# eanswer/TactileSimulation

Hardware: AMD Instinct MI355X
Metric: env-steps/sec (fwd+bwd) TactilePush batch=4096 (higher is better)
Workload: dtype f32

## Files before the change

include/tsim.h:

```cpp
#ifndef TSIM_H
#define TSIM_H
#include <stdint.h>
#ifdef __cplusplus
extern "C" {
#endif

typedef struct tsim_batch tsim_batch;
enum { TSIM_F32 = 0, TSIM_F64 = 1 };

int tsim_batch_create(const int32_t* I, const double* F, int B, int tape_capacity, int dtype, int device,
                      tsim_batch** out);
void tsim_batch_destroy(tsim_batch* b);

int tsim_ndof_r(const tsim_batch* b);
int tsim_ndof_u(const tsim_batch* b);
int tsim_ndof_var(const tsim_batch* b);
int tsim_ndof_tactile(const tsim_batch* b);
int tsim_batch_size(const tsim_batch* b);
int tsim_dtype(const tsim_batch* b);
double tsim_timestep(const tsim_batch* b);
int tsim_tape_len(const tsim_batch* b);

int tsim_update_model(tsim_batch* b, const int32_t* I, const double* F, void* stream);

int tsim_set_env_tables(tsim_batch* b, const void* tables, void* stream);
int tsim_table_size(const tsim_batch* b);

int tsim_set_param_grad(tsim_batch* b, void* dL_dtables);

enum { TSIM_PG_CONTACT = 1, TSIM_PG_INERTIAL = 2, TSIM_PG_MOTOR = 4, TSIM_PG_LIMIT = 8 };
int tsim_set_param_grad_groups(tsim_batch* b, int mask);
int tsim_get_param_grad_groups(const tsim_batch* b);

enum { TSIM_ADJ_BACKWARD = 0, TSIM_ADJ_BACKWARD_Z = 1, TSIM_ADJ_CLOSED_BACKWARD_Z = 2 };
int tsim_last_adjoint_launch(const tsim_batch* b, int32_t* out);

int tsim_reset(tsim_batch* b, const void* q0, const void* qd0, int backward_flag, void* stream);

int tsim_reset_masked(tsim_batch* b, const void* q0, const void* qd0, const int32_t* mask, void* stream);

int tsim_step(tsim_batch* b, const void* u, int num_steps, void* q_out, void* qd_out, void* var_out,
              void* tac_out, int32_t* status, void* stream);

int tsim_get_state(tsim_batch* b, void* q_out, void* qd_out, void* stream);
int tsim_readout(tsim_batch* b, void* var_out, void* tac_out, void* stream);

int tsim_backward_steps(tsim_batch* b, int n, int seed_mode, const void* df_dq, const void* df_dvar,
                        const void* df_dtac, void* df_du, void* stream);

int tsim_rollout(tsim_batch* b, const void* u, int num_frames, int num_steps, const int32_t* tactile_slot,
                 void* q_out, void* qd_out, void* var_out, void* tac_out, int32_t* status, void* stream);

int tsim_backward_episode(tsim_batch* b, int num_frames, int num_steps, const int32_t* tactile_slot,
                          const void* df_dq, const void* df_dvar, const void* df_dtac, void* df_du, void* stream);

enum { TSIM_TANGENT_MAX_DIR = 8 };
int tsim_tangent_episode(tsim_batch* b, int num_frames, int num_steps, int ndir, const int32_t* tactile_slot,
                         const void* du, const void* dq0, const void* dqd0, const void* dtables,
                         void* dq_out, void* dqd_out, void* dvar_out, void* dtac_out, void* stream);
int tsim_tangent_launch_info(const tsim_batch* b, int ndir, int with_dtables, int32_t* out);

int tsim_frame_jacobians(tsim_batch* b, int num_frames, int num_steps, void* A_out, void* B_out, void* Jvar_out, void* stream);
int tsim_frame_jacobians_launch_info(const tsim_batch* b, int32_t* out);

int tsim_tactile_jacobians(tsim_batch* b, int num_frames, int num_steps, const int32_t* tactile_slot, void* Ct_out, void* stream);
int tsim_tactile_jacobians_launch_info(const tsim_batch* b, int32_t* out);

enum { TSIM_PARAM_JACOBIAN_MAX_COLS = 32 };
int tsim_param_jacobians(tsim_batch* b, int num_frames, int num_steps, int ncols, const int32_t* cols,
                         const int32_t* tactile_slot, void* E_out, void* Ft_out, void* stream);
int tsim_param_jacobians_launch_info(const tsim_batch* b, int32_t* out);

int tsim_get_adjoint(tsim_batch* b, void* df_dq0, void* df_dqd0, void* stream);

int tsim_cache_save(tsim_batch* b, void* stream);
int tsim_cache_pop(tsim_batch* b, void* stream);
int tsim_cache_clear(tsim_batch* b);
int tsim_cache_reserve(tsim_batch* b, int depth);
int tsim_cache_depth(const tsim_batch* b);

int tsim_debug_eval(tsim_batch* b, const void* q1, const void* q0, const void* qd0, const void* u,
                    void* g_out, void* H_out, long long* cycles, void* stream);

int tsim_debug_signature(tsim_batch* b, int t_first, int n, uint32_t* out, void* stream);

int tsim_debug_stamps(tsim_batch* b, long long* cycles);

int tsim_launch_info(const tsim_batch* b, int32_t* out);
enum { TSIM_KT_FORWARD = 0, TSIM_KT_TAXELS = 1, TSIM_KT_BACKWARD = 2, TSIM_KT_COUNT = 3 };
int tsim_kernel_timing(tsim_batch* b, int enable);
int tsim_kernel_times(tsim_batch* b, double* ms_sum, int32_t* launches);
int tsim_set_lanes_per_env(tsim_batch* b, int lanes);
int tsim_static_model(const tsim_batch* b);
int tsim_set_static(tsim_batch* b, int allow);
const char* tsim_kernel_variant(const tsim_batch* b);
enum { TSIM_OPT_PAIR_CULL = 1, TSIM_OPT_VALUE_TRIALS = 2, TSIM_OPT_TRIAL_HELPERS = 3, TSIM_OPT_VALUE_FIRST = 4, TSIM_OPT_CROSS_KINKS = 5, TSIM_OPT_EVAL_BUDGET = 6,
       TSIM_OPT_ALL_DEFAULT = 7, TSIM_OPT_FRAME_RECORDS = 8, TSIM_OPT_FORWARD_SPLIT = 9 };
int tsim_set_option(tsim_batch* b, int option, int value);
int tsim_get_option(const tsim_batch* b, int option);

int tsim_last_evals(tsim_batch* b, int32_t* host_out);
int tsim_last_helper_trials(tsim_batch* b, int32_t* host_out);

#define TSIM_KINK_FACTOR 1000.0
#define TSIM_KINK_LS 4
#define TSIM_KINK_MAX 6
int tsim_set_solver_options(tsim_batch* b, int cross_kinks, int eval_budget);
int tsim_last_gnorm(tsim_batch* b, float* host_out);

const char* tsim_last_error(void);

#ifdef __cplusplus
}
#endif
#endif
```

tactilesimulation_amd/csrc/tsim_batch.h:

```cpp
#pragma once
#include <hip/hip_runtime.h>
#include <cstdint>
#include <string>
#include <vector>
#include "../../include/tsim.h"
#include "tsim_launch.h"

static thread_local std::string g_err;
static int fail(const std::string& m) { g_err = m; return 1; }
#define HIPCHK(x) do { hipError_t e_ = (x); if (e_ != hipSuccess) return fail(std::string(#x) + ": " + hipGetErrorString(e_)); } while (0)

struct DeviceGuard {
  int prev = -1; bool ok = true;
  explicit DeviceGuard(int dev) {
    if (hipGetDevice(&prev) != hipSuccess) prev = -1;
    if (prev != dev) ok = hipSetDevice(dev) == hipSuccess; else prev = -1;
  }
  ~DeviceGuard() { if (prev >= 0) (void)hipSetDevice(prev); }
};
#define TS_DEVICE(b) DeviceGuard guard_((b)->device); if (!guard_.ok) return fail("hipSetDevice(" + std::to_string((b)->device) + ") failed")

static bool capturing(hipStream_t st) {
  hipStreamCaptureStatus cs = hipStreamCaptureStatusNone;
  return hipStreamIsCapturing(st, &cs) != hipSuccess || cs != hipStreamCaptureStatusNone;
}

template <class F> static auto by_dtype(int dtype, F&& f) { return dtype == TSIM_F32 ? f(float()) : f(double()); }

struct DevBuf {
  void* p = nullptr;
  DevBuf() = default;
  DevBuf(const DevBuf&) = delete;
  DevBuf& operator=(const DevBuf&) = delete;
  ~DevBuf() { (void)hipFree(p); }
  template <class U> operator U*() const { return static_cast<U*>(p); }
  explicit operator bool() const { return p != nullptr; }
  void** operator&() { return &p; }
  void* take() { void* q = p; p = nullptr; return q; }
  void release() { (void)hipFree(take()); }
};

struct CacheEntry { void* buf; int len; int record, tape_k_ok; };
struct KtPair { hipEvent_t a, b; int kind; };
struct tsim_batch {
  int B, dtype, device, cap;
  std::vector<int32_t> I; std::vector<double> F;
  int nl, nr, nu, nvar, ntax, rec;
  int tape_k = 0, tape_k_ok = 0;
  DevBuf dI, dF;
  DevBuf dFenv; int nfrec;
  void* tape = nullptr;
  DevBuf lamq, lamv;
  DevBuf evals;
  DevBuf helped;
  DevBuf gnorm;
  int cross_kinks = 0, eval_budget = 0;
  DevBuf order; int order_valid = 0;
  DevBuf order_ep; int order_ep_n = 0;
  DevBuf prev; int has_prev = 0;
  DevBuf poseR, poseD; int nspt;
  int has_exp;
  int t_cur, record;
  int lpe_forced;
  int nsched;
  int stage_cpt;
  int n_simd;
  int last_frame_rec = 0;
  hipStream_t split_st = nullptr;
  hipEvent_t split_fork = nullptr;
  hipEvent_t split_join = nullptr;
  int last_fwd_split = 0;
  int value_trials = 2;
  int trial_helpers = 1;
  int value_first = 1;
  bool ab_no_episode_lpt = false, ab_inkernel_readout = false, ab_no_free_run = false, ab_lockstep = false, ab_taxels_per_record = false, ab_no_envtab_cpt = false, ab_no_default_opts = false, ab_inkernel_frame_out = false; int ab_bwd_lpe = 0, ab_lpt_deal = 2;
  int pair_cull = 1;
  int static_id = 0, static_exact = 0, env_struct_ok = 0, no_static = 0;
  DevBuf dKmask, dFlag;
  DevBuf fposeR, fposeD; int fpose_frames = 0;
  int pose_valid = 0;
  int pose_off = 0;
  int tt_off = 0;
  int tax_slots = 0;
  size_t esz;
  std::vector<CacheEntry> cache;
  std::vector<void*> pool;
  std::vector<void*> retired;
  long long* bwd_stamps = nullptr;
  void* dLdp = nullptr; DevBuf zbuf, pgpart; int pg_chunks = 0;
  int pg_groups = TS_PG_CONTACT; DevBuf pgbpart;
  DevBuf tan_src; size_t tan_src_reals = 0; int tan_src_captured = 0;
  DevBuf pg_slots;
  int adj_kernel = -1, adj_passes = 0;
  int kt_on = 0;
  std::vector<KtPair> kt;
  std::vector<hipEvent_t> kt_free;
};
template <class F> static auto by_real(const tsim_batch* b, F&& f) { return by_dtype(b->dtype, f); }
static void split_release(tsim_batch* b) {
  if (b->split_st) (void)hipStreamDestroy(b->split_st);
  if (b->split_fork) (void)hipEventDestroy(b->split_fork);
  if (b->split_join) (void)hipEventDestroy(b->split_join);
  b->split_st = nullptr; b->split_fork = b->split_join = nullptr;
}

struct KtScope {
  tsim_batch* b; hipStream_t st; KtPair p; bool on = false;
  KtScope(tsim_batch* b_, int kind, hipStream_t st_) : b(b_), st(st_) {
    if (!b->kt_on || b->kt.size() >= (size_t)1 << 16) return;
    if (capturing(st)) return;
    hipEvent_t e[2];
    for (int i = 0; i < 2; ++i) {
      if (!b->kt_free.empty()) { e[i] = b->kt_free.back(); b->kt_free.pop_back(); }
      else if (hipEventCreate(&e[i]) != hipSuccess) { (void)hipGetLastError(); if (i) b->kt_free.push_back(e[0]); return; }
    }
    p.a = e[0]; p.b = e[1]; p.kind = kind;
    on = hipEventRecord(p.a, st) == hipSuccess;
    if (!on) { b->kt_free.push_back(e[0]); b->kt_free.push_back(e[1]); }
  }
  ~KtScope() { if (on) { (void)hipEventRecord(p.b, st); b->kt.push_back(p); } }
};

struct GrowWant { DevBuf& buf; size_t bytes; };
static int grow_buffers(tsim_batch* b, hipStream_t st, bool named, std::initializer_list<GrowWant> want) {
  HIPCHK(hipStreamSynchronize(st));
  for (const GrowWant& w : want) {
    if (!named) w.buf.release();
    else if (w.buf) b->retired.push_back(w.buf.take());
  }
  for (const GrowWant& w : want)
    if (hipMalloc(&w.buf, w.bytes) != hipSuccess) {
      (void)hipGetLastError();
      for (const GrowWant& v : want) v.buf.release();
      return -1;
    }
  return 0;
}

static int plan_info(const TsPlan& p, int32_t* out) {
  out[0] = (int32_t)p.lds; out[1] = TS_WAVE; out[2] = (int32_t)p.grid; out[3] = p.lpe;
  return 0;
}
```

tactilesimulation_amd/csrc/tsim_hip.hip:

```cpp
#include <hip/hip_runtime.h>
#include <cstdio>
#include <cstdlib>
#include <cstring>
#include <cmath>
#include <algorithm>
#include <string>
#include <vector>
#include "../../include/tsim.h"
#include "tsim_eval.h"
#include "tsim_policy_push.h"
#include "tsim_static_pusher.h"


#include "tsim_kernels.h"
#include "tsim_param_grad.h"
#include "tsim_launch.h"
#include "tsim_batch.h"

__global__ void __launch_bounds__(1024) k_order_by_evals(const int* evals, int* order, int B, int ns, int lo, int span, int deal) {
  __shared__ int hist[64], base[64];
  const int t = threadIdx.x;
  if (t < 64) hist[t] = 0;
  __syncthreads();
  auto bin = [lo, span](int ev) { return min(max((ev - lo) * 64 / span, 0), 63); };
// ... 20 lines not shown
  const int env = blockIdx.x, lane = threadIdx.x;
  Ctx<R> c; ctx_init(c, a.I, a.F, lds, 1, 0, lane, TS_WAVE, a.stage_cpt != 0, a.Fenv ? a.Fenv + (size_t)blockIdx.x * a.fstride : nullptr);
  const int nr = c.nr, REC = ts_rec(nr, c.nu, (int)sizeof(R), a.tk);
  init_world(c, lane, TS_WAVE);
  const R* st = a.tape + ((size_t)a.t0 * a.B + env) * REC;
  if (lane < nr) { c.qD[lane] = rec_q(st)[lane]; c.q[lane] = (R)c.qD[lane]; c.qd[lane] = st[rec_qd<R>(nr) + lane]; c.qa[lane] = R(0); }
  TS_SYNC();
  phase1<R, false, true>(c, lane, R(0), R(0), R(0));
  readout<TS_WAVE>(c, lane, env, true, false, a.var_out != nullptr, false, a.var_out, (R*)nullptr);
  if (!a.poseR) return;
  int k = 0;
  for (int s = 0; s < c.nsensor; ++s) {
    const int* si = c.I + c.off_sensor + s * TSIM_SI_SIZE;
    for (int j = 0; j < si[TSIM_SI_NSPRIM]; ++j, ++k) {
      TS_SYNC();
      pair_stage_value(c, c.I[c.off_sprim + si[TSIM_SI_SPRIM0] + j], 0, lane == 0);
      TS_SYNC();
      const size_t rec = (size_t)env * a.nspt + k;
      if (lane < TP_R_SIZE) a.poseR[rec * TP_R_SIZE + lane] = c.PP[lane];
      if (lane < TP_D_SIZE) a.poseD[rec * TP_D_SIZE + lane] = c.PPd[lane];
    }
  }
}

template <class R> struct TaxArgs { const int* I; const R* F; const R* Fenv; int fstride; const R* poseR; const double* poseD; int nspt; R* tac_out; int slice;
  int B; const int* tac_slot;
  int ntax, nsensor, foff_sensor, foff_pair, foff_taxel, tt_off; };

enum { TX_MAXS = 16, TX_MAXK = 64 };
template <class R> __device__ __forceinline__ void ts_store3(R* o, R a, R b, R c) {
  __builtin_nontemporal_store(a, o); __builtin_nontemporal_store(b, o + 1); __builtin_nontemporal_store(c, o + 2);
}
template <class R>
__device__ __forceinline__ void taxel_eval(int t, V3<R> xa, int nsensor, const int* sEnd, const int* sKb, const int* sNsp, const int* sPrim, const R* sSf,
                                           const R* sShape, const R* sP, const double* sD, const R* sC, const R* tax, int ntax, R* out) {
  int s = 0;
  while (s < nsensor - 1 && t >= sEnd[s]) ++s;
  const int kb = sKb[s], nsp = sNsp[s];
  const R* sf = sSf + s * TSIM_SF_SIZE;
  const R* tp = tax + t;
  V3<R> Fl = zero3<R>();
  for (int j = 0; j < nsp; ++j) {
    const R* Cc = sC + (kb + j) * 4;
    const V3<R> dc = xa - ldv(Cc);
    if (Cc[3] >= R(0) && dot3(dc, dc) > Cc[3]) continue;
    const int prim = sPrim[kb + j];
    const R* shape = sShape + (kb + j) * 4;
    const R* P = sP + (kb + j) * TP_R_SIZE;
    const double* D = sD + (kb + j) * TP_D_SIZE;
    const M3<R> RPA = ldm(P);
    if (sizeof(R) == 4 && !(prim_distance<R>(prim, shape, mulMv(RPA, xa) + ldv(P + 9)) < R(TS_FAR_MARGIN))) continue;
    const V3<double> xPd = mulMv(ldm(D), cvt3<double>(xa)) + ldv(D + 9);
    const V3<R> xP = cvt3<R>(xPd);
    V3<R> Fc; M3<R> Jx, Jv;
    if (contact_law<R, false>(prim, shape, sf, xP, ldv(P + 15) + cross3(ldv(P + 12), xP), Fc, Jx, Jv, xPd)) Fl = Fl + mulMtv(RPA, Fc);
  }
  R o0 = R(0), o1 = R(0), o2 = R(0);
  if (Fl.x != R(0) || Fl.y != R(0) || Fl.z != R(0)) {
    o0 = Fl.x * tp[3 * ntax] + Fl.y * tp[4 * ntax] + Fl.z * tp[5 * ntax];
    o1 = Fl.x * tp[6 * ntax] + Fl.y * tp[7 * ntax] + Fl.z * tp[8 * ntax];
    o2 = Fl.x * tp[9 * ntax] + Fl.y * tp[10 * ntax] + Fl.z * tp[11 * ntax];
  }
  ts_store3(out + 3 * t, o0, o1, o2);
}
template <class R> __device__ __forceinline__ void taxel_bound(const R* P, int prim, const R* sh, R* C) {
  const V3<R> cA = mulMtv(ldm(P), ldv(P + 9)) * R(-1);
  R rb = R(-1);
  if (prim == TSIM_P_SPHERE) rb = sh[0];
  else if (prim == TSIM_P_CUBOID) rb = t_sqrt(sh[0] * sh[0] + sh[1] * sh[1] + sh[2] * sh[2]);
  else if (prim == TSIM_P_CYLINDER) rb = t_sqrt(sh[0] * sh[0] + sh[1] * sh[1]);
  C[0] = cA.x; C[1] = cA.y; C[2] = cA.z;
  C[3] = rb < R(0) ? R(-1) : (rb + R(TS_FAR_MARGIN)) * (rb + R(TS_FAR_MARGIN));
}
enum { TS_TAX_UNROLL = 2 };
template <class R>
__global__ void __launch_bounds__(256) k_taxels(TaxArgs<R> a) {
  const int rec_env = blockIdx.x, env = rec_env % a.B, frame = rec_env / a.B;
  const int tslot = a.tac_slot ? a.tac_slot[frame] : frame;
  if (tslot < 0) return;
  const int* I = a.I;
  const R* F = a.Fenv ? a.Fenv + (size_t)env * a.fstride : a.F;
  const int ntax = a.ntax, nsensor = a.nsensor;
  __shared__ int sEnd[TX_MAXS], sKb[TX_MAXS], sNsp[TX_MAXS], sPrim[TX_MAXK];
  __shared__ R sSf[TX_MAXS * TSIM_SF_SIZE], sShape[TX_MAXK * 4], sP[TX_MAXK * TP_R_SIZE];
  __shared__ double sD[TX_MAXK * TP_D_SIZE];
  __shared__ __attribute__((aligned(16))) R sC[TX_MAXK * 4];
  {
    const int* TT = I + a.tt_off;
    const int foff_sensor = a.foff_sensor, foff_pair = a.foff_pair;
    for (int i = threadIdx.x; i < nsensor; i += 256) { sEnd[i] = TT[3 * i]; sKb[i] = TT[3 * i + 1]; sNsp[i] = TT[3 * i + 2]; }
    for (int i = threadIdx.x; i < a.nspt; i += 256) sPrim[i] = TT[3 * nsensor + 2 * i];
    for (int i = threadIdx.x; i < a.nspt * 4; i += 256) sShape[i] = F[foff_pair + TT[3 * nsensor + 2 * (i >> 2) + 1] * TSIM_PF_SIZE + TSIM_PF_SHAPE + (i & 3)];
    for (int i = threadIdx.x; i < nsensor * TSIM_SF_SIZE; i += 256) sSf[i] = F[foff_sensor + i];
    for (int i = threadIdx.x; i < a.nspt * TP_R_SIZE; i += 256) sP[i] = a.poseR[(size_t)rec_env * a.nspt * TP_R_SIZE + i];
    for (int i = threadIdx.x; i < a.nspt * TP_D_SIZE; i += 256) sD[i] = a.poseD[(size_t)rec_env * a.nspt * TP_D_SIZE + i];
    __syncthreads();
    for (int k = threadIdx.x; k < a.nspt; k += 256) taxel_bound<R>(sP + k * TP_R_SIZE, sPrim[k], sShape + k * 4, sC + 4 * k);
    __syncthreads();
  }
  const R* tax = a.F + a.foff_taxel;
  R* out = a.tac_out + ((size_t)tslot * a.B + env) * 3 * ntax;
  const int te = min(ntax, ((int)blockIdx.y + 1) * a.slice);
  auto taxel = [&](int t, V3<R> xa) { taxel_eval<R>(t, xa, nsensor, sEnd, sKb, sNsp, sPrim, sSf, sShape, sP, sD, sC, tax, ntax, out); };
  if (nsensor == 1 && a.nspt == 1 && sC[3] >= R(0)) {
    enum { CH = 8 };
    __shared__ int sList[256 * CH];
    __shared__ int sCount;
    const V3<R> cA = ldv(sC);
    const R r2 = sC[3];
    const R* px = tax; const R* py = tax + ntax; const R* pz = tax + 2 * ntax;
    const int te = ntax;
    for (int base = (int)blockIdx.y * 256 * CH; base < te; base += (int)gridDim.y * 256 * CH) {
      if (threadIdx.x == 0) sCount = 0;
      __syncthreads();
      V3<R> xa[CH];
#pragma unroll
      for (int r = 0; r < CH; ++r) {
        const int tr = min(base + (int)threadIdx.x + 256 * r, te - 1);
        xa[r] = mk3<R>(px[tr], py[tr], pz[tr]);
      }
#pragma unroll
      for (int r = 0; r < CH; ++r) {
        const int tr = base + (int)threadIdx.x + 256 * r;
        if (tr < te) {
          const V3<R> dc = xa[r] - cA;
          if (dot3(dc, dc) > r2) ts_store3(out + 3 * tr, R(0), R(0), R(0));
          else sList[atomicAdd(&sCount, 1)] = tr;
        }
      }
      __syncthreads();
      const int n = sCount;
      for (int i = threadIdx.x; i < n; i += 256) {
        const int tr = sList[i];
        taxel(tr, mk3<R>(px[tr], py[tr], pz[tr]));
      }
      __syncthreads();
    }
    return;
  }
  for (int t = (int)blockIdx.y * a.slice + (int)threadIdx.x; t < te; t += 256 * TS_TAX_UNROLL) {
    V3<R> xa[TS_TAX_UNROLL];
#pragma unroll
    for (int r = 0; r < TS_TAX_UNROLL; ++r) {
      const int tr = min(t + 256 * r, te - 1);
      xa[r] = mk3<R>(tax[tr], tax[tr + ntax], tax[tr + 2 * ntax]);
    }
#pragma unroll
    for (int r = 0; r < TS_TAX_UNROLL; ++r)
      if (t + 256 * r < te) taxel(t + 256 * r, xa[r]);
  }
}

enum { TXS_RPB = 16, TXS_MAXK = 8, TXS_MAXS = 4, TXS_MAX_TAXELS = 1024 };
template <class R>
__global__ void __launch_bounds__(256) k_taxels_small(TaxArgs<R> a, int nrec, TsSubRange sub) {
  const int rec0 = blockIdx.x * TXS_RPB, nr_ = min((int)TXS_RPB, nrec - rec0);
  const int ntax = a.ntax, nsensor = a.nsensor, nspt = a.nspt;
  __shared__ int sEnd[TXS_MAXS], sKb[TXS_MAXS], sNsp[TXS_MAXS], sPrim[TXS_MAXK], sPair[TXS_MAXK], sSlot[TXS_RPB], sEnv[TXS_RPB], sRec[TXS_RPB];
  __shared__ R sSf[TXS_RPB][TXS_MAXS * TSIM_SF_SIZE], sShape[TXS_RPB][TXS_MAXK * 4], sP[TXS_RPB][TXS_MAXK * TP_R_SIZE];
  __shared__ double sD[TXS_RPB][TXS_MAXK * TP_D_SIZE];
  __shared__ __attribute__((aligned(16))) R sC[TXS_RPB][TXS_MAXK * 4];
  __shared__ R sX[3 * TXS_MAX_TAXELS];
  const R* tax = a.F + a.foff_taxel;
  for (int i = threadIdx.x; i < 3 * ntax; i += 256) sX[i] = tax[i];
  const int* TT = a.I + a.tt_off;
  for (int i = threadIdx.x; i < nsensor; i += 256) { sEnd[i] = TT[3 * i]; sKb[i] = TT[3 * i + 1]; sNsp[i] = TT[3 * i + 2]; }
  for (int i = threadIdx.x; i < nspt; i += 256) { sPrim[i] = TT[3 * nsensor + 2 * i]; sPair[i] = TT[3 * nsensor + 2 * i + 1]; }
  for (int i = threadIdx.x; i < nr_; i += 256) {
    const int fr = (rec0 + i) / sub.n, ei = sub.e0 + (rec0 + i) - fr * sub.n, env = sub.order ? sub.order[ei] : ei;
    sSlot[i] = a.tac_slot ? a.tac_slot[fr] : fr; sEnv[i] = env; sRec[i] = fr * a.B + env;
  }
  __syncthreads();
  for (int i = threadIdx.x; i < nr_ * nspt * TP_R_SIZE; i += 256) { const int r = i / (nspt * TP_R_SIZE), e = i % (nspt * TP_R_SIZE); sP[r][e] = a.poseR[(size_t)sRec[r] * nspt * TP_R_SIZE + e]; }
  for (int i = threadIdx.x; i < nr_ * nspt * TP_D_SIZE; i += 256) { const int r = i / (nspt * TP_D_SIZE), e = i % (nspt * TP_D_SIZE); sD[r][e] = a.poseD[(size_t)sRec[r] * nspt * TP_D_SIZE + e]; }
  for (int i = threadIdx.x; i < nr_ * nsensor * TSIM_SF_SIZE; i += 256) {
    const int r = i / (nsensor * TSIM_SF_SIZE), e = i % (nsensor * TSIM_SF_SIZE);
    const R* F = a.Fenv ? a.Fenv + (size_t)sEnv[r] * a.fstride : a.F;
    sSf[r][e] = F[a.foff_sensor + e];
  }
  __syncthreads();
  for (int i = threadIdx.x; i < nr_ * nspt * 4; i += 256) {
    const int r = i / (nspt * 4), e = i % (nspt * 4);
    const R* F = a.Fenv ? a.Fenv + (size_t)sEnv[r] * a.fstride : a.F;
    sShape[r][e] = F[a.foff_pair + sPair[e >> 2] * TSIM_PF_SIZE + TSIM_PF_SHAPE + (e & 3)];
  }
  __syncthreads();
  for (int i = threadIdx.x; i < nr_ * nspt; i += 256) { const int r = i / nspt, k = i % nspt; taxel_bound<R>(sP[r] + k * TP_R_SIZE, sPrim[k], sShape[r] + k * 4, sC[r] + 4 * k); }
  __syncthreads();
  for (int item = threadIdx.x; item < nr_ * ntax; item += 256) {
    const int r = item / ntax, t = item - r * ntax;
    const int tslot = sSlot[r];
    if (tslot < 0) continue;
    R* out = a.tac_out + ((size_t)tslot * a.B + sEnv[r]) * 3 * ntax;
    taxel_eval<R>(t, mk3<R>(sX[t], sX[t + ntax], sX[t + 2 * ntax]), nsensor, sEnd, sKb, sNsp, sPrim, sSf[r], sShape[r], sP[r], sD[r], sC[r], tax, ntax, out);
  }
}

template <class R> struct SigArgs { const int* I; const R* F; const R* Fenv; int fstride; int B, t_first, n; const R* tape; unsigned* out; int stage_cpt; int tk; };

__device__ __forceinline__ unsigned wave_sum_u32(unsigned x) {
  for (int off = 32; off > 0; off >>= 1) x += (unsigned)lane_gather((int)x, (int)threadIdx.x ^ off);
  return x;
}

template <class R>
__global__ void __launch_bounds__(TS_WAVE) k_signature(SigArgs<R> a) {
  extern __shared__ __attribute__((aligned(16))) unsigned char smem_raw[];
  R* lds = reinterpret_cast<R*>(smem_raw);
  const int env = blockIdx.x, lane = threadIdx.x;
  Ctx<R> c; ctx_init(c, a.I, a.F, lds, 1, 0, lane, TS_WAVE, a.stage_cpt != 0, a.Fenv ? a.Fenv + (size_t)blockIdx.x * a.fstride : nullptr);
  const int nr = c.nr, REC = ts_rec(nr, c.nu, (int)sizeof(R), a.tk);
  init_world(c, lane, TS_WAVE);
  for (int j = 0; j < a.n; ++j) {
    const R* st = a.tape + ((size_t)(a.t_first + 1 + j) * a.B + env) * REC;
    TS_SYNC();
    if (lane < nr) { c.qD[lane] = rec_q(st)[lane]; c.q[lane] = (R)c.qD[lane]; c.qd[lane] = st[rec_qd<R>(nr) + lane]; c.qa[lane] = R(0); }
    TS_SYNC();
    phase1<R, false, true>(c, lane, R(0), R(0), R(0));
    unsigned cnt = 0, sum = 0;
    for (int pk = 0; pk < c.npair; ++pk) {
      const int* pi = c.I + c.off_pair + pk * TSIM_PI_SIZE;
      if (!(pi[TSIM_PI_FLAGS] & 1)) continue;
      const R* pf = c.F + c.foff_pair + pk * TSIM_PF_SIZE;
      TS_SYNC();
      pair_stage_value(c, pk, 0, lane == 0);
      TS_SYNC();
      const R* S = c.PP;
      const M3<double> RPAd = ldm(c.PPd); const V3<double> pPAd = ldv(c.PPd + 9);
      const V3<R> wrel = ldv(S + PP_WREL), vrel = ldv(S + PP_VREL);
      for (int i = lane; i < pi[TSIM_PI_NPT]; i += TS_WAVE) {
        V3<double> xPd = mulMv(RPAd, cvt3<double>(ld_cpt(c, pi[TSIM_PI_PT0] + i))) + pPAd;
        if (pi[TSIM_PI_FLAGS] & 2) xPd.z -= (double)pf[TSIM_PF_SHAPE];
        const V3<R> xP = cvt3<R>(xPd);
        V3<R> F; M3<R> Jx, Jv; int br = 0;
        if (contact_law<R, false>(pi[TSIM_PI_PRIM], pf + TSIM_PF_SHAPE, pf + TSIM_PF_KN, xP, vrel + cross3(wrel, xP), F, Jx, Jv, xPd, &br)) {
          ++cnt; sum += ts_sig_mix((unsigned)pk, (unsigned)i, (unsigned)(1 + br));
        }
      }
    }
    for (int s = 0; s < c.nsensor; ++s) {
      const int* si = c.I + c.off_sensor + s * TSIM_SI_SIZE;
      const R* sf = c.F + c.foff_sensor + s * TSIM_SF_SIZE;
      for (int jp = 0; jp < si[TSIM_SI_NSPRIM]; ++jp) {
        const int pk = c.I[c.off_sprim + si[TSIM_SI_SPRIM0] + jp];
        const int* pi = c.I + c.off_pair + pk * TSIM_PI_SIZE;
        const R* pf = c.F + c.foff_pair + pk * TSIM_PF_SIZE;
        TS_SYNC();
        pair_stage_value(c, pk, 0, lane == 0);
        TS_SYNC();
        const R* S = c.PP;
        const V3<R> wrel = ldv(S + PP_WREL), vrel = ldv(S + PP_VREL);
        for (int i = lane; i < si[TSIM_SI_NTAX]; i += TS_WAVE) {
          const R* tp = c.Fg + c.foff_tax + si[TSIM_SI_TAX0] + i;
          const V3<double> xPd = mulMv(ldm(c.PPd), mk3<double>((double)tp[0], (double)tp[c.ntax], (double)tp[2 * c.ntax])) + ldv(c.PPd + 9);
          const V3<R> xP = cvt3<R>(xPd);
          V3<R> F; M3<R> Jx, Jv; int br = 0;
          if (contact_law<R, false>(pi[TSIM_PI_PRIM], pf + TSIM_PF_SHAPE, sf, xP, vrel + cross3(wrel, xP), F, Jx, Jv, xPd, &br)) {
            ++cnt; sum += ts_sig_mix(0x10000u + (unsigned)(si[TSIM_SI_SPRIM0] + jp), (unsigned)i, (unsigned)(1 + br));
          }
        }
      }
    }
    cnt = wave_sum_u32(cnt); sum = wave_sum_u32(sum);
    if (lane == 0) { unsigned* o = a.out + ((size_t)j * a.B + env) * 2; o[0] = cnt; o[1] = sum; }
  }
}

int tsim_fail_(const std::string& m) { return fail(m); }

static void pose_invalidate(tsim_batch* b, hipStream_t st) {
  b->pose_valid = 0;
  if (capturing(st)) b->pose_off = 1;
}


static std::vector<int32_t> build_sched(const std::vector<int32_t>& I, const std::vector<double>& F) {
  const int nl = I[TSIM_IH_NL], nr = I[TSIM_IH_NR], ol = I[TSIM_IH_OFF_LINK];
  std::vector<int> parent(nl + 1, 0), branch(nl + 1, -1), dof_link(nr, 0);
  std::vector<std::vector<int>> links;
  for (int i = 1; i <= nl; ++i) {
    const int32_t* li = &I[ol + (i - 1) * TSIM_LI_SIZE];
    parent[i] = li[TSIM_LI_PARENT];
    if (parent[i] == 0) { branch[i] = (int)links.size(); links.emplace_back(); }
    else branch[i] = branch[parent[i]];
    links[branch[i]].push_back(i);
    for (int k = li[TSIM_LI_DOF0]; k < li[TSIM_LI_DOF0] + li[TSIM_LI_NDOF]; ++k) dof_link[k] = i;
  }
  int nsteps = 0;
  for (auto& l : links) nsteps = std::max(nsteps, (int)l.size());
  std::vector<int> leader(links.size(), -1);
  for (int k = nr - 1; k >= 0; --k) leader[branch[dof_link[k]]] = k;
  const int npair = I[TSIM_IH_NPAIR], op = I[TSIM_IH_OFF_PAIR];
  const int nu = I[TSIM_IH_NU], om = I[TSIM_IH_OFF_MOTOR];
  std::vector<int32_t> S(TS_SCHED_ENT + nsteps * 16 + nl * TS_LR_SIZE + npair * TSIM_PI_SIZE + 16 + nu * TSIM_MI_SIZE, 0);
  S[0] = (int32_t)S.size(); S[1] = nsteps;
  for (int l = 0; l < 16; ++l) S[TS_SCHED_BRANCH + l] = l < nr ? branch[dof_link[l]] : -1;
  for (size_t b = 0; b < links.size() && b < 16; ++b) S[TS_SCHED_LEADER + b] = leader[b];
  S[TS_SCHED_NB] = (int32_t)links.size();
  for (int st = 0; st < nsteps; ++st)
    for (int l = 0; l < nr && l < 16; ++l) {
      const int br = branch[dof_link[l]];
      if (st < (int)links[br].size()) S[TS_SCHED_ENT + st * 16 + l] = links[br][st] | ((leader[br] == l) ? 0x100 : 0);
    }
  const int rec0 = TS_SCHED_ENT + nsteps * 16;
  for (int i = 1; i <= nl; ++i) {
    const int32_t* li = &I[ol + (i - 1) * TSIM_LI_SIZE];
    int32_t* r = &S[rec0 + (i - 1) * TS_LR_SIZE];
    r[TS_LR_PARENT] = li[TSIM_LI_PARENT]; r[TS_LR_JTYPE] = li[TSIM_LI_JTYPE]; r[TS_LR_DOF0] = li[TSIM_LI_DOF0];
    r[TS_LR_NDOF] = li[TSIM_LI_NDOF]; r[TS_LR_ANCMASK] = li[TSIM_LI_ANCMASK]; r[TS_LR_BRANCH] = branch[i];
  }
  for (int e = 0; e < npair * TSIM_PI_SIZE; ++e) S[rec0 + nl * TS_LR_SIZE + e] = I[op + e];
  {
    const int ns_ = I[TSIM_IH_NSENSOR], os = I[TSIM_IH_OFF_SENSOR], osp = I[TSIM_IH_OFF_SPRIM];
    S[TS_SCHED_TAXTAB] = (int32_t)S.size();
    int kb = 0;
    for (int s = 0; s < ns_; ++s) {
      const int32_t* si = &I[os + s * TSIM_SI_SIZE];
      S.push_back(si[TSIM_SI_TAX0] + si[TSIM_SI_NTAX]); S.push_back(kb); S.push_back(si[TSIM_SI_NSPRIM]);
      kb += si[TSIM_SI_NSPRIM];
    }
    for (int s = 0; s < ns_; ++s) {
      const int32_t* si = &I[os + s * TSIM_SI_SIZE];
      for (int j = 0; j < si[TSIM_SI_NSPRIM]; ++j) {
        const int pk = I[osp + si[TSIM_SI_SPRIM0] + j];
        S.push_back(I[op + pk * TSIM_PI_SIZE + TSIM_PI_PRIM]); S.push_back(pk);
      }
    }
    S[0] = (int32_t)S.size();
  }
  {
    S[TS_SCHED_PBOUND] = (int32_t)S.size();
    const int ncpt = I[TSIM_IH_NCPT], fc = I[TSIM_IH_FOFF_CPT];
    for (int pk = 0; pk < npair; ++pk) {
      const int32_t* pi = &I[op + pk * TSIM_PI_SIZE];
      const int p0_ = pi[TSIM_PI_PT0], n_ = pi[TSIM_PI_NPT];
      float bd[4] = {0.f, 0.f, 0.f, -1.f};
      if (n_ > 0 && !(pi[TSIM_PI_FLAGS] & 2)) {
        double lo[3], hi[3], cc[3];
        for (int a_ = 0; a_ < 3; ++a_) { lo[a_] = 1e300; hi[a_] = -1e300; }
        for (int i = 0; i < n_; ++i) for (int a_ = 0; a_ < 3; ++a_) { const double v = F[fc + a_ * ncpt + p0_ + i]; lo[a_] = std::min(lo[a_], v); hi[a_] = std::max(hi[a_], v); }
        for (int a_ = 0; a_ < 3; ++a_) { bd[a_] = (float)(0.5 * (lo[a_] + hi[a_])); cc[a_] = (double)bd[a_]; }
        double r2 = 0.0;
        for (int i = 0; i < n_; ++i) { double d2 = 0.0; for (int a_ = 0; a_ < 3; ++a_) { const double d = F[fc + a_ * ncpt + p0_ + i] - cc[a_]; d2 += d * d; } r2 = std::max(r2, d2); }
        bd[3] = (float)(std::sqrt(r2) * (1.0 + 1e-6) + 1e-7);
      }
      for (int e = 0; e < 4; ++e) { int32_t w; std::memcpy(&w, &bd[e], 4); S.push_back(w); }
    }
// ... 75 lines not shown
static int zero_async(void* p, size_t bytes, hipStream_t st) {
  const size_t n = bytes / 4;
  if (n == 0) return 0;
  hipLaunchKernelGGL(k_zero_words, dim3((unsigned)((n + 255) / 256)), dim3(256), 0, st, (uint32_t*)p, n);
  HIPCHK(hipGetLastError());
  return 0;
}

__global__ void k_check_structure(const float* tables, const float* ref, const unsigned char* km, int nfrec, size_t n, int* flag) {
  const size_t i = (size_t)blockIdx.x * blockDim.x + threadIdx.x;
  if (i >= n) return;
  const int f = (int)(i % (size_t)nfrec);
  if (km[f] && !(tables[i] == ref[f])) atomicOr(flag, 1);
}
template <class R> __global__ void k_env_header(R* tables, const R* ref, int nfrec, int B) {
  const int i = blockIdx.x * blockDim.x + threadIdx.x;
  if (i < B * TSIM_FH_SIZE) tables[(size_t)(i / TSIM_FH_SIZE) * nfrec + i % TSIM_FH_SIZE] = ref[i % TSIM_FH_SIZE];
}
template <class R> __global__ void k_set_state(R* tape, const R* q, const R* qd, int B, int nr, int rec) {
  int i = blockIdx.x * blockDim.x + threadIdx.x;
  if (i >= B * nr) return;
  int env = i / nr, k = i % nr;
  rec_q(tape + (size_t)env * rec)[k] = (double)q[i];
  tape[(size_t)env * rec + rec_qd<R>(nr) + k] = qd ? qd[i] : R(0);
}
template <class R> __global__ void k_set_state_masked(R* tape_rec, const R* q, const R* qd, const int32_t* mask, double* prev, R h, int B, int nr, int rec) {
  int i = blockIdx.x * blockDim.x + threadIdx.x;
  if (i >= B * nr) return;
  int env = i / nr, k = i % nr;
  if (!mask[env]) return;
  rec_q(tape_rec + (size_t)env * rec)[k] = (double)q[i];
  tape_rec[(size_t)env * rec + rec_qd<R>(nr) + k] = qd ? qd[i] : R(0);
  if (prev) { const double v = qd ? (double)qd[i] : 0.0; prev[(size_t)env * 2 * nr + k] = (double)q[i] - (double)h * v; prev[(size_t)env * 2 * nr + nr + k] = v; }
}
template <class R> __global__ void k_get_state(const R* tape_rec, R* q, R* qd, int B, int nr, int rec) {
  int i = blockIdx.x * blockDim.x + threadIdx.x;
  if (i >= B * nr) return;
  int env = i / nr, k = i % nr;
  if (q) q[i] = (R)rec_q(tape_rec + (size_t)env * rec)[k];
  if (qd) qd[i] = tape_rec[(size_t)env * rec + rec_qd<R>(nr) + k];
}

static size_t lds_bytes_for(const tsim_batch* b, int nslot) {
  const int reals = ts_lds_reals(b->nl, b->nr, b->nu, b->nfrec, b->I[TSIM_IH_NCPT], b->stage_cpt != 0, nslot, bool(b->dFenv), b->nsched + (int)b->I.size(), (int)b->esz);
  return ((size_t)reals * b->esz + 15) / 16 * 16;
}
struct LaunchShape { int lpe; unsigned grid; size_t lds; };
static LaunchShape launch_shape(const tsim_batch* b, int lpe_forced) {
  LaunchShape L;
  int lpe = lpe_forced;
  const size_t lds_cap = lpe_forced ? 64 * 1024 : 40 * 1024;
  if (!lpe) {
    lpe = TS_WAVE;
    double best = 1e30;
    const int cand[3] = {64, 32, 16};
    const bool fused_static = kernel_mode(b, 0) != TS_KM_GENERIC;
    const double lat_generic[3] = {1.0, 0.93, 1.02}, lat_static[3] = {1.0, 1.13, 1.24};
    const double* lat = fused_static ? lat_static : lat_generic;
    for (int i = 0; i < 3; ++i) {
      const int ns = TS_WAVE / cand[i];
      if (i > 0 && lds_bytes_for(b, ns) > lds_cap) break;
      const long long waves = ((long long)b->B + ns - 1) / ns;
      const double t = (double)((waves + b->n_simd - 1) / b->n_simd) * lat[i];
      if (t < best) { best = t; lpe = cand[i]; }
    }
  }
  if (b->has_exp) lpe = TS_WAVE;
  while (lpe < TS_WAVE && lds_bytes_for(b, TS_WAVE / lpe) > lds_cap) lpe *= 2;
  L.lpe = lpe;
  const int ns = TS_WAVE / lpe;
  L.grid = (unsigned)((b->B + ns - 1) / ns);
  L.lds = lds_bytes_for(b, ns);
  return L;
}
static void decide_stage_cpt(tsim_batch* b) {
  b->stage_cpt = 0;
  if ((size_t)3 * b->I[TSIM_IH_NCPT] * b->esz > TS_CPT_LDS_BYTES) return;
  if (b->dFenv && b->ab_no_envtab_cpt) return;
  const int lpe0 = launch_shape(b, b->lpe_forced).lpe;
  b->stage_cpt = 1;
  if (launch_shape(b, b->lpe_forced).lpe != lpe0 || lds_bytes_for(b, 1) > 64 * 1024) b->stage_cpt = 0;
}
static void shape_changed(tsim_batch* b) {
  b->order_valid = 0; b->order_ep_n = 0;
  decide_stage_cpt(b);
}
enum { TS_TAN_LDS_CAP = 64 * 1024 };
struct SlotPlan { TsPlan plan; size_t ctx_lds; };
static SlotPlan slot_block_plan(const tsim_batch* b, TsPlan p, int shape_reals, int own_reals) {
  while (p.lpe < TS_WAVE && lds_bytes_for(b, TS_WAVE / p.lpe) + (TS_WAVE / p.lpe) * ((size_t)shape_reals * b->esz) > TS_TAN_LDS_CAP) p.lpe *= 2;
  const int ns = TS_WAVE / p.lpe;
  p.grid = (unsigned)((b->B + ns - 1) / ns);
  const size_t ctx_lds = lds_bytes_for(b, ns);
  p.lds = ctx_lds + (((size_t)ns * own_reals * b->esz + 15) / 16) * 16;
  return {p, ctx_lds};
}
static TsPlan ts_plan(const tsim_batch* b, int kernel, bool policy, int lpe) {
  int forced = lpe ? lpe : b->lpe_forced;
  if (kernel == TS_K_DEBUG_EVAL && !forced) forced = TS_WAVE;
  const LaunchShape L = launch_shape(b, forced);
  TsPlan p;
  p.kernel = kernel; p.policy = policy; p.lpe = L.lpe; p.grid = L.grid; p.lds = L.lds;
  p.expj = b->has_exp; p.nrm = b->has_exp || b->nr > 8 ? 16 : 8;
  const bool adjoint = kernel == TS_K_BACKWARD || kernel == TS_K_BACKWARD_Z || kernel == TS_K_CLOSED_BACKWARD_Z;
  p.variant = kernel == TS_K_PARAM_GRAD || kernel == TS_K_PARAM_GRAD_BODY || kernel == TS_K_TANGENT || kernel == TS_K_TANGENT_BODY || kernel == TS_K_CLOSED_TANGENT || kernel == TS_K_FRAME_JACOBIAN || kernel == TS_K_TACTILE_JACOBIAN || kernel == TS_K_PARAM_JACOBIAN || (adjoint && !b->tape_k_ok) ? TS_KM_GENERIC : kernel_mode(b, forced);
  if (p.variant != TS_KM_GENERIC && !pusher_instantiated(b, kernel, policy, false, p.lpe)) p.variant = TS_KM_GENERIC;
  p.default_opts = p.variant != TS_KM_GENERIC && default_options(b) && pusher_instantiated(b, kernel, policy, true, p.lpe);
  p.fused = p.variant == TS_KM_STATIC ? ts_static_fused<TsStaticPusher, float>() : p.variant == TS_KM_PARAM && ts_static_fused<TsParamPusher, float>();
  if (kernel == TS_K_TANGENT || kernel == TS_K_CLOSED_TANGENT) {
    return slot_block_plan(b, p, ts_tan_slot_reals(b->nr, b->nu, ts_pg_count(b->I[TSIM_IH_NPAIR], b->I[TSIM_IH_NSENSOR], b->nr), 4, TS_TAN_MAX_DIR), 0).plan;
  }
  if (kernel == TS_K_FRAME_JACOBIAN) return slot_block_plan(b, p, ts_fj_slot_reals(b->nr, b->nu), 0).plan;
  if (kernel == TS_K_TACTILE_JACOBIAN) return slot_block_plan(b, p, ts_tj_slot_reals(b->nr), 0).plan;
  if (kernel == TS_K_PARAM_JACOBIAN) return slot_block_plan(b, p, ts_pj_slot_reals(b->nr), 0).plan;
  return p;
}
template <class R> static FwdArgs<R> fwd_args(const tsim_batch* b) {
  FwdArgs<R> a{};
  a.I = b->dI; a.F = (const R*)b->dF; a.Fenv = (const R*)b->dFenv; a.fstride = b->nfrec; a.B = b->B; a.record = b->record; a.t0 = b->t_cur;
  a.tape = (R*)b->tape; a.evals = b->evals; a.prev = (double*)b->prev; a.has_prev = b->has_prev; a.stage_cpt = b->stage_cpt;
  a.cross_kinks = b->cross_kinks; a.eval_budget = b->eval_budget; a.gnorm = b->gnorm; a.cull = b->pair_cull; a.vo_ls = b->value_trials;
  a.default_opts = default_options(b) ? 1 : 0; a.tk = b->tape_k;
  return a;
}
template <class R> static BwdArgs<R> bwd_args(const tsim_batch* b) {
  BwdArgs<R> a{};
  a.I = b->dI; a.F = (const R*)b->dF; a.Fenv = (const R*)b->dFenv; a.fstride = b->nfrec; a.B = b->B; a.t_end = b->t_cur;
  a.tape = (const R*)b->tape; a.lamq = (R*)b->lamq; a.lamv = (R*)b->lamv; a.stage_cpt = b->stage_cpt; a.cull = b->pair_cull; a.tk = b->tape_k;
  return a;
}

enum { TS_POSE_EMIT_MIN_TAXELS = 4096 };
static bool pose_emit(tsim_batch* b, hipStream_t st) {
  pose_invalidate(b, st);
  return !b->pose_off && b->nspt > 0 && b->poseR && b->ntax >= TS_POSE_EMIT_MIN_TAXELS;
}

static bool taxels_supported(const tsim_batch* b) { return b->ntax > 0 && b->nspt > 0 && b->nspt <= TX_MAXK && b->I[TSIM_IH_NSENSOR] <= TX_MAXS; }
static bool taxels_small(const tsim_batch* b, long long nrec) {
  return nrec >= 4 * TXS_RPB && b->ntax <= TXS_MAX_TAXELS && b->nspt <= TXS_MAXK && b->I[TSIM_IH_NSENSOR] <= TXS_MAXS && !b->ab_taxels_per_record;
}
template <class R>
static int launch_taxels(tsim_batch* b, const void* poseR, const double* poseD, int frames, const int32_t* tac_slot, void* tac_out, hipStream_t st, const TsSubRange* sub = nullptr) {
  if (b->tax_slots == 0) {
    int per_cu = 0;
    const hipError_t e_ = hipOccupancyMaxActiveBlocksPerMultiprocessor(&per_cu, k_taxels<R>, 256, 0);
    b->tax_slots = (e_ == hipSuccess && per_cu > 0 ? per_cu : 4) * (b->n_simd / 4);
  }
  const TsSubRange all{nullptr, 0, b->B};
  const long long nrec = (long long)frames * (sub ? sub->n : b->B);
  if (taxels_small(b, nrec)) {
    TaxArgs<R> t{b->dI, (const R*)b->dF, (const R*)b->dFenv, b->nfrec, (const R*)poseR, poseD, b->nspt, (R*)tac_out, 0, b->B, tac_slot,
                 b->ntax, b->I[TSIM_IH_NSENSOR], b->I[TSIM_IH_FOFF_SENSOR], b->I[TSIM_IH_FOFF_PAIR], b->I[TSIM_IH_FOFF_TAXEL], b->tt_off};
    hipLaunchKernelGGL(k_taxels_small<R>, dim3((unsigned)((nrec + TXS_RPB - 1) / TXS_RPB)), dim3(256), 0, st, t, (int)nrec, sub ? *sub : all);
    HIPCHK(hipGetLastError());
    return 0;
  }
  if (sub) return fail("launch_taxels: a sub-range of the environments is k_taxels_small's");
  const int per_env = (int)std::max<long long>(1, std::min<long long>(b->tax_slots / nrec, (b->ntax + 255) / 256));
  const int slice = ((b->ntax + per_env - 1) / per_env + 255) / 256 * 256;
  const dim3 tgrid((unsigned)nrec, (b->ntax + slice - 1) / slice);
  TaxArgs<R> t{b->dI, (const R*)b->dF, (const R*)b->dFenv, b->nfrec, (const R*)poseR, poseD, b->nspt, (R*)tac_out, slice, b->B, tac_slot,
               b->ntax, b->I[TSIM_IH_NSENSOR], b->I[TSIM_IH_FOFF_SENSOR], b->I[TSIM_IH_FOFF_PAIR], b->I[TSIM_IH_FOFF_TAXEL], b->tt_off};
  hipLaunchKernelGGL(k_taxels<R>, tgrid, dim3(256), 0, st, t);
  HIPCHK(hipGetLastError());
  return 0;
}

template <class R>
static int launch_forward(tsim_batch* b, const void* u, int nframes, const int32_t* tac_slot, int nsub, void* q_out, void* qd_out, void* var_out, void* tac_out, int32_t* status, hipStream_t st) {
  FwdArgs<R> a = fwd_args<R>(b);
  a.nsub = nsub; a.nframes = nframes; a.tac_slot = tac_slot; a.u = (const R*)u;
  a.q_out = (R*)q_out; a.qd_out = (R*)qd_out; a.var_out = (R*)var_out; a.tac_out = (R*)tac_out; a.status = status;
  a.order = (b->B >= 256 && nframes == 1 && b->order_valid) ? (const int*)b->order : (b->B >= 256 && nframes > 1 && b->order_ep_n == nframes * nsub && !b->ab_no_episode_lpt) ? (const int*)b->order_ep : nullptr;
  a.vo_first = b->value_first; a.helpers = b->trial_helpers; a.helped = b->helped;
  const bool emit = pose_emit(b, st);
  a.nspt = b->nspt;
  if (emit) { a.poseR = (R*)b->poseR; a.poseD = b->poseD; }
  const size_t fpose_bytes = (size_t)nframes * b->B * (size_t)std::max(b->nspt, 1) * (TP_R_SIZE * b->esz + TP_D_SIZE * sizeof(double));
  bool defer = tac_out && taxels_supported(b) && fpose_bytes <= ((size_t)1 << 30) && !b->ab_inkernel_readout;
  if (defer && b->fpose_frames < nframes) {
    if (capturing(st)) defer = false;
    else {
      const size_t nrec = (size_t)nframes * b->B * b->nspt;
      const int rc = grow_buffers(b, st, b->pose_off != 0, {{b->fposeR, nrec * TP_R_SIZE * b->esz}, {b->fposeD, nrec * TP_D_SIZE * sizeof(double)}});
      if (rc > 0) return rc;
      b->fpose_frames = rc ? 0 : nframes;
      if (rc) defer = false;
    }
  }
  if (defer) { a.fposeR = (R*)b->fposeR; a.fposeD = b->fposeD; }
  a.free_run = (defer || !tac_out || b->ntax == 0) && !b->ab_no_free_run;
  a.lockstep = b->ab_lockstep ? 1 : 0;
  if (a.lockstep) a.free_run = 0;
  TsPlan plan = ts_plan(b, TS_K_FORWARD, false, 0);
  if (b->record && !plan.fused) b->tape_k_ok = 0;
  const TsPlan fr_plan = ts_plan(b, TS_K_FRAME_RECORDS, false, 0);
  const bool frame_rec = defer && a.free_run && b->record && nframes > 1 && plan.fused && !emit && !b->ab_inkernel_frame_out &&
                         fr_plan.variant == plan.variant && fr_plan.lpe == plan.lpe;
  a.frame_rec = frame_rec ? 1 : 0;
  plan.frame_rec = frame_rec;
  b->last_frame_rec = !frame_rec ? 0 : (plan.frame_rec && plan.default_opts) ? 2 : 1;
  const int ns_ = TS_WAVE / plan.lpe;
  auto frame_records = [&](hipStream_t s, const TsSubRange& sub) {
    TsPlan p = fr_plan;
    const int nblk = (sub.n + ns_ - 1) / ns_, chunks = std::max(1, std::min(nframes, b->n_simd / std::max(nblk, 1))), fpc = (nframes + chunks - 1) / chunks;
    p.grid = (unsigned)(nblk * ((nframes + fpc - 1) / fpc));
    return ts_launch<false, R>(p, s, a, fpc, sub);
  };
  const int nblk_f = (int)plan.grid, wh = std::max(1, nblk_f / 8);
  const bool split = frame_rec && b->split_st && a.order && a.order == (const int*)b->order_ep && b->B % ns_ == 0 && nblk_f <= b->n_simd && nblk_f >= 64 &&
                     taxels_small(b, (long long)nframes * wh * ns_) && !capturing(st);
  b->last_fwd_split = split ? 1 : 0;
  if (split) {
    const TsSubRange heavy{a.order, 0, wh * ns_}, light{a.order, wh * ns_, b->B - wh * ns_};
    auto forward = [&](hipStream_t s, unsigned grid, const FwdArgs<R>& fa) -> int {
      TsPlan p = plan; p.grid = grid;
      if (!ts_launch<false, R>(p, s, fa)) return fail("no k_forward instantiation for the launch plan");
      HIPCHK(hipGetLastError());
      return 0;
    };
    auto read_out = [&](hipStream_t s, const TsSubRange& sub) -> int {
      if (!frame_records(s, sub)) return fail("no k_frame_records instantiation for the launch plan");
      HIPCHK(hipGetLastError());
      return launch_taxels<R>(b, b->fposeR, b->fposeD, nframes, tac_slot, tac_out, s, &sub);
    };
    int rc;
    {
      KtScope kt_(b, TSIM_KT_FORWARD, st);
      HIPCHK(hipEventRecord(b->split_fork, st));
      HIPCHK(hipStreamWaitEvent(b->split_st, b->split_fork, 0));
      rc = forward(st, (unsigned)wh, a);
    }
    if (!rc) {
      FwdArgs<R> al = a; al.order = a.order + light.e0;
      rc = forward(b->split_st, (unsigned)(nblk_f - wh), al);
    }
    if (!rc) rc = read_out(b->split_st, light);
    const hipError_t e_rec = hipEventRecord(b->split_join, b->split_st);
    hipError_t e_wait;
    {
      KtScope kt_(b, TSIM_KT_TAXELS, st);
      if (!rc) rc = read_out(st, heavy);
      e_wait = e_rec == hipSuccess ? hipStreamWaitEvent(st, b->split_join, 0) : hipStreamSynchronize(b->split_st);
    }
    if (rc) return rc;
    HIPCHK(e_rec);
    HIPCHK(e_wait);
  } else {
    { KtScope kt_(b, TSIM_KT_FORWARD, st); if (!ts_launch<false, R>(plan, st, a)) return fail("no k_forward instantiation for the launch plan"); }
    HIPCHK(hipGetLastError());
    if (defer) {
      KtScope kt_(b, TSIM_KT_TAXELS, st);
      if (frame_rec) {
        if (!frame_records(st, TsSubRange{nullptr, 0, b->B})) return fail("no k_frame_records instantiation for the launch plan");
        HIPCHK(hipGetLastError());
      }
      if (launch_taxels<R>(b, b->fposeR, b->fposeD, nframes, tac_slot, tac_out, st)) return 1;
    }
  }
  b->pose_valid = emit ? 1 : 0;
  if (b->B >= 256) {
    const int ns = TS_WAVE / plan.lpe, nsv = (b->B % ns == 0) ? ns : 1;
    if (nframes > 1) {
      const int n = nframes * nsub;
      hipLaunchKernelGGL(k_order_by_evals, dim3(1), dim3(1024), 0, st, (const int*)b->evals, b->order_ep, b->B, nsv, 2 * n, std::max(1, 5 * n / 2), b->ab_lpt_deal);
      b->order_ep_n = n; b->order_valid = 0;
    } else {
      hipLaunchKernelGGL(k_order_by_evals, dim3(1), dim3(1024), 0, st, (const int*)b->evals, b->order, b->B, nsv, 0, 64, b->ab_lpt_deal);
      b->order_valid = 1;
    }
    HIPCHK(hipGetLastError());
  } else if (nframes > 1) b->order_valid = 0;
  return 0;
}

struct PgLayout { int nchunk, chunk_len, most; };
static PgLayout pg_layout(const tsim_batch* b, int n) {
  const int want = (int)std::max<long long>(1, (16LL * b->n_simd + b->B - 1) / b->B);
  const int most = std::max(1, std::min(n, want)), chunk_len = (n + most - 1) / most;
  return {(n + chunk_len - 1) / chunk_len, chunk_len, most};
}
template <class R> static void pg_common(const tsim_batch* b, PgCommon<R>& p, int n, int nchunk, int chunk_len) {
  p.I = b->dI; p.F = (const R*)b->dF; p.Fenv = (const R*)b->dFenv; p.fstride = b->nfrec; p.B = b->B; p.n = n; p.t_end = b->t_cur;
  p.tape = (const R*)b->tape; p.nchunk = nchunk; p.chunk_len = chunk_len; p.stage_cpt = b->stage_cpt; p.tk = b->tape_k;
}
template <class R, class Args>
static int launch_param_pass(tsim_batch* b, TsKernel kernel, const char* name, const char* no_part, Args& p, int n, void* part, const PgSeg (&seg)[3], hipStream_t st) {
  const PgLayout lay = pg_layout(b, n);
  pg_common<R>(b, p, n, lay.nchunk, lay.chunk_len);
  p.z = (const R*)b->zbuf; p.P = seg[0].count + seg[1].count + seg[2].count; p.part = (R*)part;
  if (!part || p.nchunk > b->pg_chunks) return fail(no_part);
  TsPlan plan = ts_plan(b, kernel, false, 0);
  plan.grid *= p.nchunk;
  if (!TsLaunch<void, false, R>::run(plan, st, p)) return fail(std::string("no ") + name + " instantiation for the launch plan");
  HIPCHK(hipGetLastError());
  ts_param_reduce_launch(PgReduceArgs<R>{(const R*)part, p.nchunk, b->B, p.P, (R*)b->dLdp, b->nfrec, {seg[0], seg[1], seg[2]}}, st);
  HIPCHK(hipGetLastError());
  return 0;
}
template <class R>
static int launch_param_grad(tsim_batch* b, int n, int seed_stride, int frames, const int32_t* tac_slot, const void* df_dtac, hipStream_t st) {
  PgArgs<R> p;
  p.seed_stride = seed_stride; p.frames = frames; p.tac_slot = tac_slot; p.df_dtac = (const R*)df_dtac;
  const PgSeg seg[3] = {{4 * b->I[TSIM_IH_NPAIR], 4, TSIM_PF_SIZE, b->I[TSIM_IH_FOFF_PAIR] + TSIM_PF_KN, 1},
                        {4 * b->I[TSIM_IH_NSENSOR], 4, TSIM_SF_SIZE, b->I[TSIM_IH_FOFF_SENSOR] + TSIM_SF_KN, 1},
                        {b->nr, 1, TSIM_DF_SIZE, b->I[TSIM_IH_FOFF_DOF] + TSIM_DF_DAMPING, 1}};
  return launch_param_pass<R>(b, TS_K_PARAM_GRAD, "k_param_grad", "param_grad: partial-sum buffer too small", p, n, b->pgpart, seg, st);
}
template <class R>
static int launch_param_grad_body(tsim_batch* b, int n, hipStream_t st) {
  PgBodyArgs<R> p;
  p.groups = b->pg_groups;
  const PgSeg seg[3] = {{10 * b->I[TSIM_IH_NL], 10, TSIM_LF_SIZE, b->I[TSIM_IH_FOFF_LINK] + TSIM_LF_MASS, b->pg_groups & TS_PG_INERTIAL},
                        {4 * b->nu, 4, 4, b->I[TSIM_IH_FOFF_MOTOR], b->pg_groups & TS_PG_MOTOR},
                        {3 * b->nr, 3, TSIM_DF_SIZE, b->I[TSIM_IH_FOFF_DOF] + TSIM_DF_LIM_LO, b->pg_groups & TS_PG_LIMIT}};
  return launch_param_pass<R>(b, TS_K_PARAM_GRAD_BODY, "k_param_grad_body", "param_grad: the body groups' partial-sum buffer is missing or too small", p, n,
                              b->pgbpart, seg, st);
}

template <class R>
static int launch_param_passes(tsim_batch* b, int n, int seed_stride, int frames, const int32_t* tac_slot, const void* df_dtac, hipStream_t st) {
  b->adj_passes = 0;
  if (!b->dLdp) return 0;
  if (b->pg_groups & TS_PG_CONTACT) {
    if (launch_param_grad<R>(b, n, seed_stride, frames, tac_slot, df_dtac, st)) return 1;
    b->adj_passes |= 1;
  }
  if (b->pg_groups & ~TS_PG_CONTACT) {
    if (launch_param_grad_body<R>(b, n, st)) return 1;
    b->adj_passes |= 2;
  }
  return 0;
}

template <class R>
static int launch_backward(tsim_batch* b, int n, int seed_stride, int frames, const int32_t* tac_slot, const void* df_dq, const void* df_dvar, const void* df_dtac, void* df_du, hipStream_t st) {
  BwdArgs<R> a = bwd_args<R>(b);
  a.n = n; a.seed_stride = seed_stride; a.frames = frames; a.tac_slot = tac_slot;
  a.df_dq = (const R*)df_dq; a.df_dvar = (const R*)df_dvar; a.df_dtac = (const R*)df_dtac; a.df_du = (R*)df_du; a.cyc = b->bwd_stamps;
  {
    KtScope kt_(b, TSIM_KT_BACKWARD, st);
    const TsPlan plan = ts_plan(b, b->dLdp ? TS_K_BACKWARD_Z : TS_K_BACKWARD, false, b->ab_bwd_lpe);
    if (!ts_launch<false, R>(plan, st, a, (R*)b->zbuf)) return fail("no k_backward instantiation for the launch plan");
  }
  HIPCHK(hipGetLastError());
  b->adj_kernel = b->dLdp ? TSIM_ADJ_BACKWARD_Z : TSIM_ADJ_BACKWARD;
  return launch_param_passes<R>(b, n, seed_stride, frames, tac_slot, df_dtac, st);
}

static SlotPlan tangent_plan(const tsim_batch* b, int ndir, bool with_dtab, int kernel = TS_K_TANGENT) {
  const int nhist = b->I[TSIM_IH_INTEGRATOR] == 2 ? 4 : 2, P = with_dtab ? ts_pg_count(b->I[TSIM_IH_NPAIR], b->I[TSIM_IH_NSENSOR], b->nr) : 0;
  return slot_block_plan(b, ts_plan(b, kernel, false, 0), 0, ts_tan_slot_reals(b->nr, b->nu, P, nhist, ndir));
}
template <class R>
static void tangent_args(const tsim_batch* b, TanArgs<R>& a, int T, int S, int ndir, const int32_t* tac_slot, const void* du, const void* dq0, const void* dqd0, const void* dtab,
                         void* dq_out, void* dqd_out, void* dvar_out, void* dtac_out) {
  a.I = b->dI; a.F = (const R*)b->dF; a.Fenv = (const R*)b->dFenv; a.fstride = b->nfrec;
  a.B = b->B; a.n = T * S; a.t_end = b->t_cur; a.nsub = S; a.nframes = T; a.ndir = ndir; a.tk = b->tape_k;
  a.stage_cpt = b->stage_cpt; a.cull = b->pair_cull; a.tac_slot = tac_slot; a.tape = (const R*)b->tape;
  a.du = (const R*)du; a.dq0 = (const R*)dq0; a.dqd0 = (const R*)dqd0; a.dtab = (const R*)dtab;
  a.dq_out = (R*)dq_out; a.dqd_out = (R*)dqd_out; a.dvar_out = (R*)dvar_out; a.dtac_out = (R*)dtac_out;
}
template <class R>
static int launch_tangent_body_src(tsim_batch* b, TanArgs<R>& a, hipStream_t st, const char* who) {
  if (!a.dtab || !(b->pg_groups & ~TS_PG_CONTACT)) return 0;
  const int ndir = a.ndir;
  const size_t need = (size_t)ndir * a.n * b->B * b->nr;
  const bool cap = capturing(st);
  if (need > b->tan_src_reals) {
    if (cap)
      return fail(std::string(who) + ": the body columns' workspace must grow, which a stream capture cannot do: call once with these sizes before capturing");
    const int rc = grow_buffers(b, st, b->tan_src_captured != 0, {{b->tan_src, need * b->esz}});
    if (rc > 0) return rc;
    b->tan_src_captured = 0;
    b->tan_src_reals = rc ? 0 : need;
    if (rc) return fail(std::string(who) + ": hipMalloc of the body columns' workspace failed");
  }
  const PgLayout lay = pg_layout(b, a.n);
  TanBodyArgs<R> p{};
  pg_common<R>(b, p, a.n, lay.nchunk, lay.chunk_len);
  p.groups = b->pg_groups; p.ndir = ndir; p.dtab = a.dtab; p.src = (R*)b->tan_src;
  if (cap) b->tan_src_captured = 1;
  TsPlan bp = ts_plan(b, TS_K_TANGENT_BODY, false, 0);
  bp.grid *= p.nchunk;
  if (!TsLaunch<void, false, R>::run(bp, st, p)) return fail("no k_tangent_body_src instantiation for the launch plan");
  HIPCHK(hipGetLastError());
  a.src = (const R*)b->tan_src;
  return 0;
}
template <class R>
static int launch_tangent(tsim_batch* b, int T, int S, int ndir, const int32_t* tac_slot, const void* du, const void* dq0, const void* dqd0, const void* dtab,
                          void* dq_out, void* dqd_out, void* dvar_out, void* dtac_out, hipStream_t st) {
  TanArgs<R> a{};
  tangent_args<R>(b, a, T, S, ndir, tac_slot, du, dq0, dqd0, dtab, dq_out, dqd_out, dvar_out, dtac_out);
  const auto [plan, ctx_lds] = tangent_plan(b, ndir, dtab != nullptr);
  a.xoff = (int)(ctx_lds / b->esz);
  if (plan.lds > TS_TAN_LDS_CAP) return fail("tangent_episode: the tangent state of " + std::to_string(ndir) + " directions does not fit the block's LDS for this model");
  if (int rc = launch_tangent_body_src<R>(b, a, st, "tangent_episode")) return rc;
  if (!(a.src ? TsLaunch<void, false, R>::run_tangent_src(plan, st, a) : TsLaunch<void, false, R>::run(plan, st, a))) return fail("no k_tangent instantiation for the launch plan");
  HIPCHK(hipGetLastError());
  return 0;
}

static SlotPlan frame_jacobian_plan(const tsim_batch* b) { return slot_block_plan(b, ts_plan(b, TS_K_FRAME_JACOBIAN, false, 0), 0, ts_fj_slot_reals(b->nr, b->nu)); }
template <class R>
static int launch_frame_jacobians(tsim_batch* b, int T, int S, void* A_out, void* B_out, void* Jvar_out, hipStream_t st) {
  auto [plan, ctx_lds] = frame_jacobian_plan(b);
  if (plan.lds > TS_TAN_LDS_CAP) return fail("frame_jacobians: the " + std::to_string(ts_fj_ncol(b->nr, b->nu)) + " columns of an environment do not fit the block's LDS for this model");
  if ((unsigned long long)plan.grid * (unsigned)T > 0x7fffffffull) return fail("frame_jacobians: too many blocks");
  FjArgs<R> a{};
  pg_common<R>(b, a, T * S, T, S);
  a.cull = b->pair_cull; a.xoff = (int)(ctx_lds / b->esz);
  a.A_out = (R*)A_out; a.B_out = (R*)B_out; a.Jvar_out = (R*)Jvar_out;
  plan.grid *= (unsigned)T;
  if (!TsLaunch<void, false, R>::run(plan, st, a)) return fail("no k_frame_jacobian instantiation for the launch plan");
  HIPCHK(hipGetLastError());
  return 0;
}

static SlotPlan tactile_jacobian_plan(const tsim_batch* b) { return slot_block_plan(b, ts_plan(b, TS_K_TACTILE_JACOBIAN, false, 0), 0, ts_tj_slot_reals(b->nr)); }
template <class R>
static int launch_tactile_jacobians(tsim_batch* b, int T, int S, const int32_t* tac_slot, void* Ct_out, hipStream_t st) {
  auto [plan, ctx_lds] = tactile_jacobian_plan(b);
  if (plan.lds > TS_TAN_LDS_CAP) return fail("tactile_jacobians: a pair's per-dof records do not fit the block's LDS next to the context for this model");
  if ((unsigned long long)plan.grid * (unsigned)T > 0x7fffffffull) return fail("tactile_jacobians: too many blocks");
  TjArgs<R> a{};
  pg_common<R>(b, a, T * S, T, S);
  a.cull = b->pair_cull; a.xoff = (int)(ctx_lds / b->esz);
  a.tac_slot = tac_slot; a.Ct_out = (R*)Ct_out;
  plan.grid *= (unsigned)T;
  if (!TsLaunch<void, false, R>::run(plan, st, a)) return fail("no k_tactile_jacobian instantiation for the launch plan");
  HIPCHK(hipGetLastError());
  return 0;
}

static SlotPlan param_jacobian_plan(const tsim_batch* b) { return slot_block_plan(b, ts_plan(b, TS_K_PARAM_JACOBIAN, false, 0), 0, ts_pj_slot_reals(b->nr)); }
template <class R>
static int launch_param_jacobians(tsim_batch* b, int T, int S, int ncols, const int* cidx, const int32_t* tac_slot, void* E_out, void* Ft_out, hipStream_t st) {
  auto [plan, ctx_lds] = param_jacobian_plan(b);
  if (plan.lds > TS_TAN_LDS_CAP) return fail("param_jacobians: the " + std::to_string((int)TS_PJ_MAX_COLS) + " columns of an environment do not fit the block's LDS for this model");
  if ((unsigned long long)plan.grid * (unsigned)T > 0x7fffffffull) return fail("param_jacobians: too many blocks");
  PjArgs<R> a{};
  pg_common<R>(b, a, T * S, T, S);
  a.cull = b->pair_cull; a.xoff = (int)(ctx_lds / b->esz);
  a.ncols = ncols;
  for (int k = 0; k < ncols; ++k) a.col[k] = cidx[k];
  a.tac_slot = tac_slot; a.E_out = (R*)E_out; a.Ft_out = (R*)Ft_out;
  plan.grid *= (unsigned)T;
  if (!TsLaunch<void, false, R>::run(plan, st, a)) return fail("no k_param_jacobian instantiation for the launch plan");
  HIPCHK(hipGetLastError());
  return 0;
}

static int frames_positive(const std::string& who, int num_frames, int num_steps) {
  return num_frames <= 0 || num_steps <= 0 ? fail(who + ": num_frames and num_steps must be positive") : 0;
}
static int taped_window(const tsim_batch* b, const std::string& who, int num_frames, int num_steps, long long* n) {
  if (int rc = frames_positive(who, num_frames, num_steps)) return rc;
  *n = (long long)num_frames * num_steps;
  return *n > b->t_cur ? fail(who + ": only " + std::to_string(b->t_cur) + " sub-steps on the tape") : 0;
}
static int bdf2_window_is_the_tape(const tsim_batch* b, const std::string& who, long long n) {
  if (b->I[TSIM_IH_INTEGRATOR] != 2 || n == b->t_cur) return 0;
  return fail(who + ": a BDF2 model's window must start at tape record 0 (no tangent is carried across calls); the tape holds " + std::to_string(b->t_cur) + " sub-steps");
}

extern "C" {

const char* tsim_last_error(void) { return g_err.c_str(); }

int tsim_batch_create(const int32_t* I, const double* F, int B, int tape_capacity, int dtype, int device, tsim_batch** out) {
  if (!I || !F || !out) return fail("null argument");
  if (I[TSIM_IH_MAGIC] != TSIM_MAGIC || I[TSIM_IH_VERSION] != TSIM_VERSION) return fail("model blob: bad magic/version");
  if (B <= 0 || tape_capacity < 0) return fail("bad batch size / tape capacity");
  if (dtype != TSIM_F32 && dtype != TSIM_F64) return fail("bad dtype");
  if (I[TSIM_IH_INTEGRATOR] != 1 && I[TSIM_IH_INTEGRATOR] != 2) return fail("unknown integrator");
  const int nl = I[TSIM_IH_NL], nr = I[TSIM_IH_NR], nu = I[TSIM_IH_NU];
  int n_exp = 0;
  if (nr > 16 || nr < 1 || nu > 16) return fail("ndof_r must be in 1..16 and ndof_u <= 16");
  for (int i = 1; i <= nl; ++i) {
    int jt = I[I[TSIM_IH_OFF_LINK] + (i - 1) * TSIM_LI_SIZE + TSIM_LI_JTYPE];
    if (jt != TSIM_J_REVOLUTE && jt != TSIM_J_PRISMATIC && jt != TSIM_J_PLANAR && jt != TSIM_J_TRANSLATIONAL && jt != TSIM_J_SPHERICAL_EXP)
      return fail("joint type not supported by the HIP path");
    if (jt == TSIM_J_SPHERICAL_EXP && ++n_exp > 1) return fail("at most one rotation-vector joint per model on the HIP path");
  }
  for (int s = 0; s < I[TSIM_IH_NSENSOR]; ++s)
    if (I[I[TSIM_IH_OFF_SENSOR] + s * TSIM_SI_SIZE + TSIM_SI_NSPRIM] > 16) return fail("too many primitives per sensor");
  DeviceGuard guard_(device);
  if (!guard_.ok) return fail("hipSetDevice(" + std::to_string(device) + ") failed");
  tsim_batch* b = new tsim_batch();
  b->B = B; b->dtype = dtype; b->device = device; b->cap = tape_capacity;
  b->I.assign(I, I + I[TSIM_IH_NI]); b->F.assign(F, F + I[TSIM_IH_NF]);
  b->nl = nl; b->nr = nr; b->nu = nu; b->nvar = I[TSIM_IH_NVAR]; b->ntax = I[TSIM_IH_NTAXEL];
  b->esz = dtype == TSIM_F32 ? 4 : 8;
  b->t_cur = 0; b->record = 0; b->has_exp = n_exp > 0;
  b->nfrec = I[TSIM_IH_FOFF_CPT];
  b->lpe_forced = 0;
  { const std::vector<int32_t> S_ = build_sched(b->I, b->F); b->nsched = (int)S_.size(); b->tt_off = b->I[TSIM_IH_NI] + S_[TS_SCHED_TAXTAB]; }
  b->pair_cull = getenv("TSIM_NO_PAIR_CULL") ? 0 : 1;
  b->no_static = getenv("TSIM_NO_STATIC") != nullptr;
  b->trial_helpers = getenv("TSIM_NO_TRIAL_HELPERS") ? 0 : 1;
  b->ab_no_episode_lpt = getenv("TSIM_NO_EPISODE_LPT") != nullptr; b->ab_inkernel_readout = getenv("TSIM_INKERNEL_READOUT") != nullptr;
  b->ab_no_free_run = getenv("TSIM_NO_FREE_RUN") != nullptr; b->ab_lockstep = getenv("TSIM_LOCKSTEP") != nullptr; b->ab_no_default_opts = getenv("TSIM_NO_DEFAULT_OPTS") != nullptr;
  if (const char* e = getenv("TSIM_LPT_DEAL")) b->ab_lpt_deal = atoi(e);
  if (const char* e = getenv("TSIM_BWD_LPE")) { const int v = atoi(e); if (v == 16 || v == 32 || v == 64) b->ab_bwd_lpe = v; }
  b->ab_taxels_per_record = getenv("TSIM_TAXELS_PER_RECORD") != nullptr; b->ab_no_envtab_cpt = getenv("TSIM_NO_ENVTAB_CPT") != nullptr;
  b->value_first = getenv("TSIM_NO_VALUE_FIRST") ? 0 : 1;
  b->ab_inkernel_frame_out = getenv("TSIM_INKERNEL_FRAME_OUT") != nullptr;
  if (const char* e = getenv("TSIM_VALUE_TRIALS")) b->value_trials = std::max(0, atoi(e));
  if (const char* e = getenv("TSIM_LPE")) { const int v = atoi(e); if (v == 16 || v == 32 || v == 64) b->lpe_forced = v; }
  b->cross_kinks = dtype == TSIM_F32 ? 1 : 0;
  {
    int cus = 0;
    if (hipDeviceGetAttribute(&cus, hipDeviceAttributeMultiprocessorCount, device) != hipSuccess || cus <= 0) cus = 256;
    b->n_simd = 4 * cus;
  }
  b->stage_cpt = 0;
  detect_static_model(b);
  b->tape_k = kernel_mode(b, b->lpe_forced) != TS_KM_GENERIC ? 1 : 0;
  b->rec = ts_rec(nr, nu, (int)b->esz, b->tape_k);
  if (lds_bytes_for(b, 1) > 64 * 1024) { delete b; return fail("model needs more than 64 KiB of LDS per environment"); }
  decide_stage_cpt(b);
  b->nspt = b->I[TSIM_IH_NSPRIM];
  size_t tape_bytes = (size_t)(tape_capacity + 1) * B * b->rec * b->esz;
  if (hipMalloc(&b->dI, (b->I.size() + b->nsched) * sizeof(int32_t)) != hipSuccess || hipMalloc(&b->dF, b->F.size() * b->esz) != hipSuccess ||
      hipMalloc(&b->tape, tape_bytes) != hipSuccess || hipMalloc(&b->lamq, (size_t)2 * B * nr * b->esz) != hipSuccess ||
      hipMalloc(&b->lamv, (size_t)2 * B * nr * b->esz) != hipSuccess || hipMalloc(&b->evals, (size_t)B * sizeof(int)) != hipSuccess || hipMalloc((void**)&b->helped, (size_t)B * sizeof(int)) != hipSuccess || hipMemset(b->helped, 0, (size_t)B * sizeof(int)) != hipSuccess || hipMalloc((void**)&b->gnorm, (size_t)B * sizeof(float)) != hipSuccess || hipMalloc(&b->order, (size_t)B * sizeof(int)) != hipSuccess || hipMalloc((void**)&b->order_ep, (size_t)B * sizeof(int)) != hipSuccess || hipMalloc(&b->prev, (size_t)B * 2 * nr * sizeof(double)) != hipSuccess ||
      (b->nspt > 0 && (hipMalloc(&b->poseR, (size_t)B * b->nspt * TP_R_SIZE * b->esz) != hipSuccess || hipMalloc((void**)&b->poseD, (size_t)B * b->nspt * TP_D_SIZE * sizeof(double)) != hipSuccess))) {
    tsim_batch_destroy(b);
    return fail("hipMalloc failed (tape bytes = " + std::to_string(tape_bytes) + ")");
  }
  if (hipMemset(b->tape, 0, tape_bytes) != hipSuccess || hipMemset(b->lamq, 0, (size_t)2 * B * nr * b->esz) != hipSuccess ||
      hipMemset(b->lamv, 0, (size_t)2 * B * nr * b->esz) != hipSuccess) { tsim_batch_destroy(b); return fail("hipMemset failed"); }
  if (upload_model(b, nullptr)) { tsim_batch_destroy(b); return 1; }
  if (B >= 64 && !getenv("TSIM_NO_FORWARD_SPLIT")) {
    if (hipStreamCreateWithFlags(&b->split_st, hipStreamNonBlocking) != hipSuccess || hipEventCreateWithFlags(&b->split_fork, hipEventDisableTiming) != hipSuccess ||
        hipEventCreateWithFlags(&b->split_join, hipEventDisableTiming) != hipSuccess) {
      (void)hipGetLastError();
      split_release(b);
    }
  }
  *out = b;
  return 0;
}

void tsim_batch_destroy(tsim_batch* b) {
  if (!b) return;
  DeviceGuard guard_(b->device);
  for (auto& e : b->cache) (void)hipFree(e.buf);
  for (void* p : b->pool) (void)hipFree(p);
  for (void* p : b->retired) (void)hipFree(p);
  for (auto& k : b->kt) { (void)hipEventDestroy(k.a); (void)hipEventDestroy(k.b); }
  for (hipEvent_t e : b->kt_free) (void)hipEventDestroy(e);
  split_release(b);
  (void)hipFree(b->tape);
  delete b;
}

int tsim_ndof_r(const tsim_batch* b) { return b->nr; }
int tsim_ndof_u(const tsim_batch* b) { return b->nu; }
int tsim_ndof_var(const tsim_batch* b) { return 3 * b->nvar; }
int tsim_ndof_tactile(const tsim_batch* b) { return 3 * b->ntax; }
int tsim_batch_size(const tsim_batch* b) { return b->B; }
int tsim_dtype(const tsim_batch* b) { return b->dtype; }
double tsim_timestep(const tsim_batch* b) { return b->F[TSIM_FH_H]; }
int tsim_tape_len(const tsim_batch* b) { return b->record ? b->t_cur : 0; }
int tsim_launch_info(const tsim_batch* b, int32_t* out) { return plan_info(ts_plan(b, TS_K_FORWARD, false, 0), out); }
int tsim_tangent_launch_info(const tsim_batch* b, int ndir, int with_dtables, int32_t* out) {
  if (!b || !out) return fail("tangent_launch_info: null argument");
  if (ndir < 1 || ndir > TSIM_TANGENT_MAX_DIR) return fail("tangent_launch_info: ndir must be 1 .. " + std::to_string((int)TSIM_TANGENT_MAX_DIR));
  return plan_info(tangent_plan(b, ndir, with_dtables != 0).plan, out);
}
int tsim_frame_jacobians_launch_info(const tsim_batch* b, int32_t* out) {
  if (!b || !out) return fail("frame_jacobians_launch_info: null argument");
  return plan_info(frame_jacobian_plan(b).plan, out);
}
int tsim_tactile_jacobians_launch_info(const tsim_batch* b, int32_t* out) {
  if (!b || !out) return fail("tactile_jacobians_launch_info: null argument");
  return plan_info(tactile_jacobian_plan(b).plan, out);
}
int tsim_param_jacobians_launch_info(const tsim_batch* b, int32_t* out) {
  if (!b || !out) return fail("param_jacobians_launch_info: null argument");
  return plan_info(param_jacobian_plan(b).plan, out);
}
int tsim_kernel_timing(tsim_batch* b, int enable) { b->kt_on = enable ? 1 : 0; return 0; }
int tsim_kernel_times(tsim_batch* b, double* ms_sum, int32_t* launches) {
  if (!ms_sum || !launches) return fail("kernel_times: null argument");
  TS_DEVICE(b);
  for (int k = 0; k < TSIM_KT_COUNT; ++k) { ms_sum[k] = 0.0; launches[k] = 0; }
  for (auto& p : b->kt) {
    float ms = 0.f;
    HIPCHK(hipEventSynchronize(p.b));
    HIPCHK(hipEventElapsedTime(&ms, p.a, p.b));
    ms_sum[p.kind] += ms; launches[p.kind] += 1;
    b->kt_free.push_back(p.a); b->kt_free.push_back(p.b);
  }
  b->kt.clear();
  return 0;
}
int tsim_set_lanes_per_env(tsim_batch* b, int lanes) {
  if (lanes != 0 && lanes != 16 && lanes != 32 && lanes != 64) return fail("set_lanes_per_env: 0 (automatic), 16, 32 or 64");
  b->lpe_forced = lanes;
  shape_changed(b);
  return 0;
}
int tsim_static_model(const tsim_batch* b) { return kernel_mode(b, b->lpe_forced) != TS_KM_GENERIC ? b->static_id : 0; }
const char* tsim_kernel_variant(const tsim_batch* b) {
  const int km = kernel_mode(b, b->lpe_forced);
  if (km == TS_KM_STATIC) return "static:pusher";
  if (km == TS_KM_PARAM) return "param:pusher";
  return "generic";
}
int tsim_set_static(tsim_batch* b, int allow) {
  b->no_static = allow ? 0 : 1;
  shape_changed(b);
  return 0;
}
int tsim_set_option(tsim_batch* b, int option, int value) {
  if (option == TSIM_OPT_PAIR_CULL) { b->pair_cull = value != 0; return 0; }
  if (option == TSIM_OPT_VALUE_TRIALS) { if (value < 0) return fail("set_option: TSIM_OPT_VALUE_TRIALS >= 0"); b->value_trials = value; return 0; }
  if (option == TSIM_OPT_TRIAL_HELPERS) { b->trial_helpers = value != 0; return 0; }
  if (option == TSIM_OPT_VALUE_FIRST) { b->value_first = value != 0; return 0; }
  return fail("set_option: unknown option " + std::to_string(option));
}
int tsim_get_option(const tsim_batch* b, int option) {
  if (option == TSIM_OPT_PAIR_CULL) return b->pair_cull;
  if (option == TSIM_OPT_VALUE_TRIALS) return b->value_trials;
  if (option == TSIM_OPT_TRIAL_HELPERS) return b->trial_helpers;
  if (option == TSIM_OPT_VALUE_FIRST) return b->value_first;
  if (option == TSIM_OPT_CROSS_KINKS) return b->cross_kinks;
  if (option == TSIM_OPT_EVAL_BUDGET) return b->eval_budget;
  if (option == TSIM_OPT_ALL_DEFAULT) return default_options(b) ? 1 : 0;
  if (option == TSIM_OPT_FRAME_RECORDS) return b->last_frame_rec;
  if (option == TSIM_OPT_FORWARD_SPLIT) return b->last_fwd_split;
  return -1;
}
int tsim_set_solver_options(tsim_batch* b, int cross_kinks, int eval_budget) {
  if (eval_budget < 0) return fail("set_solver_options: negative evaluation budget");
  b->cross_kinks = cross_kinks != 0;
  b->eval_budget = eval_budget;
  return 0;
}
int tsim_last_gnorm(tsim_batch* b, float* host_out) {
  TS_DEVICE(b);
  if (hipMemcpy(host_out, b->gnorm, (size_t)b->B * sizeof(float), hipMemcpyDeviceToHost) != hipSuccess) return fail("last_gnorm: copy failed");
  return 0;
}
int tsim_last_helper_trials(tsim_batch* b, int32_t* host_out) {
  TS_DEVICE(b);
  if (hipMemcpy(host_out, b->helped, (size_t)b->B * sizeof(int), hipMemcpyDeviceToHost) != hipSuccess) return fail("last_helper_trials: copy failed");
  return 0;
}
int tsim_last_evals(tsim_batch* b, int32_t* host_out) {
  TS_DEVICE(b);
  if (hipMemcpy(host_out, b->evals, (size_t)b->B * sizeof(int), hipMemcpyDeviceToHost) != hipSuccess) return fail("last_evals: copy failed");
  return 0;
}

int tsim_update_model(tsim_batch* b, const int32_t* I, const double* F, void* stream) {
  if (I[TSIM_IH_NI] != (int)b->I.size() || I[TSIM_IH_NF] != (int)b->F.size()) return fail("update_model: blob size changed");
  for (int i = 0; i < TSIM_IH_SIZE; ++i) if (I[i] != b->I[i]) return fail("update_model: topology changed");
  TS_DEVICE(b);
  pose_invalidate(b, (hipStream_t)stream);
  b->I.assign(I, I + I[TSIM_IH_NI]); b->F.assign(F, F + I[TSIM_IH_NF]);
  if (b->dFenv) { HIPCHK(hipFree(b->dFenv)); (void)b->dFenv.take(); b->env_struct_ok = 0; }
  if (int rc = upload_model(b, (hipStream_t)stream)) return rc;
  shape_changed(b);
  return 0;
}

int tsim_set_env_tables(tsim_batch* b, const void* tables, void* stream) {
  TS_DEVICE(b);
  pose_invalidate(b, (hipStream_t)stream);
  if (!tables) { if (b->dFenv) { HIPCHK(hipFree(b->dFenv)); (void)b->dFenv.take(); b->env_struct_ok = 0; decide_stage_cpt(b); } return 0; }
  size_t bytes = (size_t)b->B * b->nfrec * b->esz;
  const bool fresh = !b->dFenv;
  if (fresh) HIPCHK(hipMalloc(&b->dFenv, bytes));
  HIPCHK(hipMemcpyAsync(b->dFenv, tables, bytes, hipMemcpyDeviceToDevice, (hipStream_t)stream));
  {
    const unsigned nh = (unsigned)((b->B * TSIM_FH_SIZE + 255) / 256);
    by_real(b, [&](auto r) { using R = decltype(r); hipLaunchKernelGGL(k_env_header<R>, dim3(nh), dim3(256), 0, (hipStream_t)stream, (R*)b->dFenv, (const R*)b->dF, b->nfrec, b->B); });
    HIPCHK(hipGetLastError());
  }
  const int ok_before = b->env_struct_ok;
  b->env_struct_ok = 0;
  if (b->static_id != 0 && b->dtype == TSIM_F32 && !capturing((hipStream_t)stream)) {
    if (!b->dKmask) {
      std::vector<unsigned char> km(b->nfrec);
      for (int i = 0; i < b->nfrec; ++i) km[i] = TsParam<TsStaticPusher>::Fk(i) ? 1 : 0;
      HIPCHK(hipMalloc((void**)&b->dKmask, km.size())); HIPCHK(hipMalloc((void**)&b->dFlag, sizeof(int)));
      HIPCHK(hipMemcpy(b->dKmask, km.data(), km.size(), hipMemcpyHostToDevice));
    }
    int flag = 0;
    HIPCHK(hipMemsetAsync(b->dFlag, 0, sizeof(int), (hipStream_t)stream));
    const size_t n = (size_t)b->B * b->nfrec;
    hipLaunchKernelGGL(k_check_structure, dim3((unsigned)((n + 255) / 256)), dim3(256), 0, (hipStream_t)stream, (const float*)b->dFenv, (const float*)b->dF, b->dKmask, b->nfrec, n, b->dFlag);
    HIPCHK(hipGetLastError());
    HIPCHK(hipMemcpyAsync(&flag, b->dFlag, sizeof(int), hipMemcpyDeviceToHost, (hipStream_t)stream));
    HIPCHK(hipStreamSynchronize((hipStream_t)stream));
    b->env_struct_ok = flag == 0;
  }
  if (fresh || ok_before != b->env_struct_ok) shape_changed(b);
  return 0;
}
int tsim_table_size(const tsim_batch* b) { return b->nfrec; }

static int pg_alloc(tsim_batch* b) {
  const bool body = (b->pg_groups & ~TS_PG_CONTACT) != 0;
  if (b->zbuf && b->pgpart && b->pg_slots && (b->pgbpart || !body)) return 0;
  TS_DEVICE(b);
  const int chunks = pg_layout(b, b->cap).most;
  auto get = [&](void** p, size_t reals) {
    if (*p || hipMalloc(p, std::max<size_t>(reals * b->B * b->esz, 8)) == hipSuccess) return true;
    (void)hipGetLastError(); *p = nullptr;
    return false;
  };
  if (body && !get(&b->pgbpart, (size_t)chunks * ts_pgb_count(b->I[TSIM_IH_NL], b->nu, b->nr))) return fail("set_param_grad_groups: hipMalloc failed");
  if (!get(&b->zbuf, (size_t)b->cap * b->nr) || !get(&b->pgpart, (size_t)chunks * ts_pg_count(b->I[TSIM_IH_NPAIR], b->I[TSIM_IH_NSENSOR], b->nr))) {
    b->zbuf.release(); b->pgpart.release();
    return fail("set_param_grad: hipMalloc failed");
  }
  b->pg_chunks = chunks;
  if (!b->pg_slots && hipMalloc((void**)&b->pg_slots, std::max<size_t>((size_t)b->cap * sizeof(int32_t), 8)) != hipSuccess) {
    (void)hipGetLastError(); (void)b->pg_slots.take();
    return fail("set_param_grad: hipMalloc failed");
  }
  return 0;
}

int tsim_set_param_grad_groups(tsim_batch* b, int mask) {
  if (!b) return fail("set_param_grad_groups: null batch");
  if (mask < 0 || (mask & ~(TS_PG_CONTACT | TS_PG_INERTIAL | TS_PG_MOTOR | TS_PG_LIMIT))) return fail("set_param_grad_groups: unknown group in mask " + std::to_string(mask));
  const int before = b->pg_groups;
  b->pg_groups = mask;
  if (b->dLdp && pg_alloc(b)) { b->pg_groups = before; return 1; }
  return 0;
}
int tsim_get_param_grad_groups(const tsim_batch* b) { return b ? b->pg_groups : -1; }
int tsim_last_adjoint_launch(const tsim_batch* b, int32_t* out) {
  if (!b || !out) return fail("last_adjoint_launch: null argument");
  out[0] = b->adj_kernel; out[1] = b->adj_passes;
  return 0;
}

int tsim_set_param_grad(tsim_batch* b, void* dL_dtables) {
  if (dL_dtables && pg_alloc(b)) return 1;
  b->dLdp = dL_dtables;
  return 0;
}

int tsim_reset(tsim_batch* b, const void* q0, const void* qd0, int backward_flag, void* stream) {
  if (!q0) return fail("reset: q0 is null");
  TS_DEVICE(b);
  hipStream_t st = (hipStream_t)stream;
  int n = b->B * b->nr, blk = 256, grd = (n + blk - 1) / blk;
  by_real(b, [&](auto r) { using R = decltype(r); hipLaunchKernelGGL(k_set_state<R>, dim3(grd), dim3(blk), 0, st, (R*)b->tape, (const R*)q0, (const R*)qd0, b->B, b->nr, b->rec); });
  HIPCHK(hipGetLastError());
  if (zero_async(b->lamq, (size_t)2 * b->B * b->nr * b->esz, st) || zero_async(b->lamv, (size_t)2 * b->B * b->nr * b->esz, st)) return 1;
  b->t_cur = 0; b->record = backward_flag ? 1 : 0; b->order_valid = 0; b->has_prev = 0; b->tape_k_ok = b->tape_k;
  pose_invalidate(b, st);
  return 0;
}

int tsim_reset_masked(tsim_batch* b, const void* q0, const void* qd0, const int32_t* mask, void* stream) {
  if (!q0 || !mask) return fail("reset_masked: q0 / mask is null");
  if (b->record) return fail("reset_masked: not while recording (the tape is shared by the batch): use reset");
  TS_DEVICE(b);
  hipStream_t st = (hipStream_t)stream;
  pose_invalidate(b, st);
  int n = b->B * b->nr, blk = 256, grd = (n + blk - 1) / blk;
  size_t off = (size_t)b->t_cur * b->B * b->rec;
  double* prev = (b->I[TSIM_IH_INTEGRATOR] == 2 && b->has_prev) ? (double*)b->prev : nullptr;
  by_real(b, [&](auto r) {
    using R = decltype(r);
    hipLaunchKernelGGL(k_set_state_masked<R>, dim3(grd), dim3(blk), 0, st, (R*)b->tape + off, (const R*)q0, (const R*)qd0, mask, prev, (R)b->F[TSIM_FH_H], b->B, b->nr, b->rec);
  });
  HIPCHK(hipGetLastError());
  return 0;
}

int tsim_step(tsim_batch* b, const void* u, int num_steps, void* q_out, void* qd_out, void* var_out, void* tac_out, int32_t* status, void* stream) {
  if (num_steps <= 0) return fail("step: num_steps must be positive");
  if (!u && b->nu > 0) return fail("step: u is null");
  if (b->record && b->t_cur + num_steps > b->cap) return fail("step: tape capacity exceeded (" + std::to_string(b->cap) + " sub-steps)");
  TS_DEVICE(b);
  if (int rc = by_real(b, [&](auto r) { return launch_forward<decltype(r)>(b, u, 1, nullptr, num_steps, q_out, qd_out, var_out, tac_out, status, (hipStream_t)stream); })) return rc;
  if (b->record) b->t_cur += num_steps;
// ... 226 lines not shown
```

tactilesimulation_amd/csrc/tsim_kernels.h:

```cpp
#pragma once
#include <hip/hip_runtime.h>
#include "../../include/tsim.h"
#include "tsim_eval.h"
#include "tsim_policy_push.h"

template <class MS, class C> __device__ __forceinline__ int ts_integrator(const C& c) {
  if constexpr (std::is_void<MS>::value) return ts_u(c.I[TSIM_IH_INTEGRATOR]); else return MS::Iv(TSIM_IH_INTEGRATOR);
}
template <class MS> constexpr int ts_static_nr() { if constexpr (std::is_void<MS>::value) return 0; else return MS::Iv(TSIM_IH_NR); }

__host__ __device__ inline int ts_qw(int esz) { return 8 / esz; }
__host__ __device__ inline int ts_rec(int nr, int nu, int esz, int tk) { return (ts_qw(esz) * nr + nr + nr * nr + nu + (tk ? nr * nr : 0) + 1) & ~1; }
template <class R> __device__ __forceinline__ double* rec_q(R* rec) { return reinterpret_cast<double*>(rec); }
template <class R> __device__ __forceinline__ const double* rec_q(const R* rec) { return reinterpret_cast<const double*>(rec); }
template <class R> __device__ __forceinline__ int rec_qd(int nr) { return ts_qw((int)sizeof(R)) * nr; }
template <class R> __device__ __forceinline__ int rec_H(int nr) { return ts_qw((int)sizeof(R)) * nr + nr; }
template <class R> __device__ __forceinline__ int rec_u(int nr) { return ts_qw((int)sizeof(R)) * nr + nr + nr * nr; }
template <class R> __device__ __forceinline__ int rec_K(int nr, int nu) { return ts_qw((int)sizeof(R)) * nr + nr + nr * nr + nu; }

template <int LPE, class R>
__device__ __forceinline__ void readout(const Ctx<R>& c, int lane, int env, bool wr_var, bool wr, bool has_var, bool has_tac, R* var_out, R* tac_out, int tb = 0, int te = 0x7fffffff) {
  if (has_var && wr_var) {
    for (int e = lane; e < c.nvar; e += LPE) {
      const int l = c.I[c.off_var + e * TSIM_VI_SIZE + TSIM_VI_LINK];
// ... 319 lines not shown
      return true;
    };
    if (!fin && !done && !wait_) {
      bool halved = judge(gnew, 0, slot);
      if (TS_UNLIKELY(nh > 0)) {
#pragma unroll 1
        for (int j = 1; halved && j <= nh; ++j) {
          const R gj = (NS > 3 && j == 3) ? gh2 : (NS > 2 && j == 2) ? gh1 : gh0;
          const int hj = (NS > 3 && j == 3) ? hs2 : (NS > 2 && j == 2) ? hs1 : hs0;
          ++helped;
          halved = judge(gj, j, hj);
        }
      }
      if (take) {
        if (vfirst && ls >= 0) kq = (ls == 0 && !forced && gn > R(0)) ? gtake / (gn * gn) : R(1e30);
        forced = false;
        if (ls >= 0) ++iter;
        gn = gtake;
        if (!ts_finite(gn)) { nonfinite = true; fin = true; }
        else if (gn < c.tol) { conv = true; fin = true; }
        else if (iter >= c.max_iter || (TS_OPT(eval_budget, 0) > 0 && sub_evals >= TS_OPT(eval_budget, 0))) fin = true;
        else {
          solve = true;
          if (lane < nr) { c.rhs[lane] = -c.g[lane]; dlbase[lane] = c.dl[lane]; }
        }
      }
    }
    TS_SYNC();
    if (__any(solve)) {
      solve_newton<R, NRM, LPE, double, ts_static_nr<MS>()>(c.H, c.rhs, c.dq, nr, false, lane, solve);
      if (solve) {
        alpha = R(1); ls = 0;
        vo = vfirst && kq * gn * gn < R(0.25) * c.tol;
        if (lane < nr) c.dl[lane] = dlbase[lane] + c.dq[lane];
      }
      TS_SYNC();
    }
    bool commit = fin && !done && !held;
    if (TS_OPT(lockstep, 0) && !__all(fin || done)) commit = false;
    if (!free_run) {
      if (commit && s == a.nsub - 1) { held = true; commit = false; }
      if (__all(held || done)) { commit = held; held = false; }
    }
    bool frame_end = false;
    if (commit) {
      if (!conv) ++bad;
      gmax = t_max(gmax, gn);
      if (TS_RECORD && valid) {
        R* rec = a.tape + ((size_t)(a.t0 + f * a.nsub + s + 1) * a.B + env) * REC;
        if (lane < nr) { rec_q(rec)[lane] = c.qD[lane]; rec[rec_qd<R>(nr) + lane] = c.qd[lane]; }
        for (int e = lane; e < nr * nr; e += LPE) rec[rec_H<R>(nr) + e] = c.H[e];
        if (lane < nu) rec[rec_u<R>(nr) + lane] = c.u[lane];
        if constexpr (ts_static_fused<MS, R>()) { if (a.tk) for (int e = lane; e < nr * nr; e += LPE) rec[rec_K<R>(nr, nu) + e] = c.H2[e]; }
      }
      TS_SYNC();
      if (lane < nr) {
        c.qm1[lane] = c.q0[lane]; c.qm1D[lane] = c.q0D[lane]; c.qdm1[lane] = c.qd0[lane];
        c.q0[lane] = c.q[lane]; c.q0D[lane] = c.qD[lane]; c.qd0[lane] = c.qd[lane];
      }
      has_prev = true;
      fin = false; ss = true;
      if (++s == a.nsub) { s = 0; frame_end = true; }
    }
    TS_SYNC();
    if constexpr (kFrameRec) {
      if (frame_end) { ++f; fs = true; if (f == a.nframes) { done = true; fs = false; ss = false; } }
    } else if (TS_UNLIKELY(__any(frame_end))) {
#ifdef TS_ROUND_STATS
      ++fe_execs_; const long long fe_t0_ = clock64();
#endif
      if (!(ts_static_fused<MS, R>() && !POLICY && a.frame_rec != 0)) ts_frame_outputs<LPE, R, MS>(c, a, lane, env, f, tslot, frame_end, valid);
      if (frame_end) { ++f; fs = true; if (f == a.nframes) { done = true; fs = false; ss = false; } }
      TS_SYNC();
#ifdef TS_ROUND_STATS
      fe_cycles_ += clock64() - fe_t0_;
#endif
    }
  }
  if constexpr (ts_static_fused<MS, R>() && !kFrameRec) { if (a.poseR && a.nframes <= 0) ts_static_value_records<R, MS>(c, lane); }
  if (!kFrameRec && a.poseR) {
    int k = 0;
    for (int s = 0; s < c.nsensor; ++s) {
      const int* si = c.I + c.off_sensor + s * TSIM_SI_SIZE;
      const int nsp = ts_u(si[TSIM_SI_NSPRIM]), sp0 = ts_u(si[TSIM_SI_SPRIM0]);
      for (int j = 0; j < nsp; ++j, ++k) {
        TS_SYNC();
        pair_stage_value(c, ts_u(c.I[c.off_sprim + sp0 + j]), 0, lane == 0);
        TS_SYNC();
        const size_t rec = (size_t)env * a.nspt + k;
        if (valid) {
          for (int e = lane; e < TP_R_SIZE; e += LPE) a.poseR[rec * TP_R_SIZE + e] = c.PP[e];
          if (lane < TP_D_SIZE) a.poseD[rec * TP_D_SIZE + lane] = c.PPd[lane];
        }
      }
    }
  }
  if (valid) {
    if (bdf2_model && lane < nr) { a.prev[(size_t)env * 2 * nr + lane] = c.qm1D[lane]; a.prev[(size_t)env * 2 * nr + nr + lane] = (double)c.qdm1[lane]; }
    if (!TS_RECORD) {
      R* st = a.tape + ((size_t)a.t0 * a.B + env) * REC;
      if (lane < nr) { rec_q(st)[lane] = c.q0D[lane]; st[rec_qd<R>(nr) + lane] = c.qd0[lane]; }
    }
    if (a.status && lane == 0) a.status[env] = bad | (nonfinite ? (1 << 30) : 0);
    if (a.evals && lane == 0) a.evals[env] = evals;
    if (a.helped && lane == 0) a.helped[env] = helped;
    if (a.gnorm && lane == 0) a.gnorm[env] = (float)gmax;
#ifdef TS_PP_TIME
    if (a.gnorm && lane == 0) a.gnorm[env] = (float)((double)pp_cycles_ / (double)(clock64() - pp_t0_));
#endif
#ifdef TS_ROUND_STATS
    if (lane == 0) { if (a.gnorm) a.gnorm[env] = (float)(clock64() - rs_t0_); if (a.status) a.status[env] = rounds_; }
    if (lane == 0 && a.helped) a.helped[env] = (int)(fe_cycles_ < (1ll << 23) - 1 ? fe_cycles_ : (1ll << 23) - 1) * 256 + (fe_execs_ < 255 ? fe_execs_ : 255);
#endif
  }
}
#undef helpers_on
#undef TS_OPT
#undef TS_RECORD
template <class R, int NRM, bool EXPJ, int LPE, bool POLICY = false, class MS = void>
__global__ void TS_KLB k_forward(FwdArgs<R> a) { ts_forward<R, NRM, EXPJ, LPE, POLICY, MS>(a); }
template <class R, int NRM, int LPE, class MS>
__global__ void TS_KLB k_forward_fr(FwdArgs<R> a) { ts_forward<R, NRM, false, LPE, false, TsFrameRecords<TsDefaultOpts<MS>>>(a); }

template <class R, int LPE, class MS>
__global__ void TS_KLB k_frame_records(FwdArgs<R> a, int fpc, TsSubRange sub) {
  extern __shared__ __attribute__((aligned(16))) unsigned char smem_raw[];
  R* lds = reinterpret_cast<R*>(smem_raw);
  constexpr int NS = TS_WAVE / LPE;
  const int slot = threadIdx.x / LPE, lane = threadIdx.x % LPE;
  const int nblk = (sub.n + NS - 1) / NS, chunk = blockIdx.x / nblk;
  const int eidx = (blockIdx.x - chunk * nblk) * NS + slot;
  const bool valid = eidx < sub.n;
  const int ei = sub.e0 + min(eidx, sub.n - 1);
  const int env = sub.order ? sub.order[ei] : ei;
  Ctx<R> c; ctx_init<R, MS>(c, a.I, a.F, lds, NS, slot, lane, LPE, false, a.Fenv ? a.Fenv + (size_t)env * a.fstride : nullptr);
  const int nr = c.nr, REC = ts_rec(nr, c.nu, (int)sizeof(R), a.tk);
  init_world(c, lane, LPE);
  const int f0 = chunk * fpc, f1 = min(f0 + fpc, a.nframes);
  double qn = 0.0; R qdn = R(0);
  const R* st = a.tape + ((size_t)(a.t0 + (f0 + 1) * a.nsub) * a.B + env) * REC;
  const size_t frame_stride = (size_t)a.nsub * a.B * REC;
  if (f0 < f1 && lane < nr) { qn = rec_q(st)[lane]; qdn = st[rec_qd<R>(nr) + lane]; }
  for (int f = f0; f < f1; ++f) {
    const int tslot = a.tac_slot ? a.tac_slot[f] : f;
    TS_SYNC();
    if (lane < nr) { c.qD[lane] = qn; c.q0D[lane] = qn; c.q[lane] = (R)qn; c.qd[lane] = qdn; c.qd0[lane] = qdn; c.qa[lane] = R(0); }
    st += frame_stride;
    if (f + 1 < f1 && lane < nr) { qn = rec_q(st)[lane]; qdn = st[rec_qd<R>(nr) + lane]; }
    TS_SYNC();
    ts_frame_outputs<LPE, R, MS>(c, a, lane, env, f, tslot, true, valid);
  }
}


template <class R, int LPE, class MS> __device__ __forceinline__ void ts_static_output_vjp(const Ctx<R>& c, int lane, const R* wvar, const R* wtac);
template <class R> struct BwdArgs {
  const int* I; const R* F; const R* Fenv; int fstride;
  int B, n, t_end;
  int tk = 0;
  int seed_stride;
  int frames;
  const int* tac_slot;
  const R* tape;
  const R *df_dq, *df_dvar, *df_dtac;
  R *lamq, *lamv, *df_du;
  int stage_cpt;
  long long* cyc;
  PushPolicy<R> pol;
  int cull = 0;
};

template <int LPE, class R>
__device__ __forceinline__ R mass_times_z(const Ctx<R>& c, int lane) {
  const int* LR = c.LI + ts_sched_rec(c.LI);
  R* fi = c.PT;
  for (int i = 1 + lane; i <= c.nl; i += LPE) {
    const int anc = LR[(i - 1) * TS_LR_SIZE + TS_LR_ANCMASK];
    S6<R> A = zero6<R>();
    for (int k = 0; k < c.nr; ++k)
      if ((anc >> k) & 1) A = A + ld6(c.WP + k * 6) * c.z[k];
    const R* X = c.LP + i * LK_SIZE;
    st6(fi + i * 6, imul(c.F[c.foff_link + (i - 1) * TSIM_LF_SIZE + TSIM_LF_MASS], ldv(X + LK_C), X + LK_IC, A));
  }
  TS_SYNC();
  R tau = R(0);
  if (lane < c.nr) {
    const S6<R> Wj = ld6(c.WP + lane * 6);
    for (int i = 1; i <= c.nl; ++i)
      if ((LR[(i - 1) * TS_LR_SIZE + TS_LR_ANCMASK] >> lane) & 1) tau += dot6(Wj, ld6(fi + i * 6));
  }
  TS_SYNC();
  return tau;
}

template <int LPE, class R, int PRIMC = -1>
__device__ __forceinline__ bool vjp_taxels(const Ctx<R>& c, int lane, int t0, int nt, int prim, const R* shape, const R* sf, const PairPose<R>& P, const R* wtac, R (&g)[12]) {
  const M3<R> RPA = P.RPA;
  const V3<R> pPA = P.pPA, wrel = P.wrel, vrel = P.vrel;
#pragma unroll
  for (int e = 0; e < 12; ++e) g[e] = R(0);
  bool any_live = false;
  R nw0 = R(0), nw1 = R(0), nw2 = R(0), nx0 = R(0), nx1 = R(0), nx2 = R(0);
  if (lane < nt) {
    const int t = t0 + lane; const R* tp = c.Fg + c.foff_tax + t;
    nw0 = wtac[3 * t]; nw1 = wtac[3 * t + 1]; nw2 = wtac[3 * t + 2]; nx0 = tp[0]; nx1 = tp[c.ntax]; nx2 = tp[2 * c.ntax];
  }
  for (int base = 0; base < nt; base += LPE) {
    const bool valid = base + lane < nt;
    const int t = t0 + (valid ? base + lane : 0);
    const R* tp = c.Fg + c.foff_tax + t;
    const R w0 = valid ? nw0 : R(0), w1 = valid ? nw1 : R(0), w2 = valid ? nw2 : R(0);
    const R x0 = nx0, x1 = nx1, x2 = nx2;
    if (base + LPE + lane < nt) {
      const int tn = t0 + base + LPE + lane; const R* tq = c.Fg + c.foff_tax + tn;
      nw0 = wtac[3 * tn]; nw1 = wtac[3 * tn + 1]; nw2 = wtac[3 * tn + 2]; nx0 = tq[0]; nx1 = tq[c.ntax]; nx2 = tq[2 * c.ntax];
    }
    bool live = valid && (w0 != R(0) || w1 != R(0) || w2 != R(0));
    if (PRIMC >= 0 && sizeof(R) == 4 && live) live = prim_distance<R>(prim, shape, mulMv(RPA, mk3<R>(x0, x1, x2)) + pPA) < R(TS_FAR_MARGIN);
    V3<R> xP, F; M3<R> Jx, Jv;
    if (live) {
      const V3<double> xPd = mulMv(P.RPAd, mk3<double>((double)x0, (double)x1, (double)x2)) + P.pPAd;
      xP = cvt3<R>(xPd);
      live = contact_law<R, true>(prim, shape, sf, xP, vrel + cross3(wrel, xP), F, Jx, Jv, xPd);
    }
    if (!__any(live)) continue;
    any_live = true;
    if (live) {
      const V3<R> wl = mk3<R>(w0 * tp[3 * c.ntax] + w1 * tp[6 * c.ntax] + w2 * tp[9 * c.ntax],
                              w0 * tp[4 * c.ntax] + w1 * tp[7 * c.ntax] + w2 * tp[10 * c.ntax],
                              w0 * tp[5 * c.ntax] + w1 * tp[8 * c.ntax] + w2 * tp[11 * c.ntax]);
      const V3<R> wP = mulMv(RPA, wl);
      const V3<R> gv = mulMtv(Jv, wP);
      const V3<R> gx = mulMtv(Jx, wP) + cross3(gv, wrel);
      const V3<R> ath = cross3(xP, gx) + cross3(wP, F);
      const V3<R> bw = cross3(xP, gv);
      g[0] += ath.x; g[1] += ath.y; g[2] += ath.z; g[3] += gx.x; g[4] += gx.y; g[5] += gx.z;
      g[6] += bw.x; g[7] += bw.y; g[8] += bw.z; g[9] += gv.x; g[10] += gv.y; g[11] += gv.z;
    }
  }
  return any_live;
}

template <int LPE, class R>
__device__ __forceinline__ void output_vjp(const Ctx<R>& c, int lane, const R* wvar, const R* wtac) {
  const int nr = c.nr;
  if (wvar && lane < nr) {
    R acc = R(0);
    const S6<R> Wk = ld6(c.WP + lane * 6);
    for (int e = 0; e < c.nvar; ++e) {
      const int l = c.I[c.off_var + e * TSIM_VI_SIZE + TSIM_VI_LINK];
      if (!((anc_of(c.I, c.off_link, l) >> lane) & 1)) continue;
      const V3<R> x = mulMv(ldm(c.LP + l * LK_SIZE + LK_R), ldv(c.F + c.foff_var + e * TSIM_VF_SIZE)) + ldv(c.LP + l * LK_SIZE + LK_P);
      const V3<R> J = cross3(Wk.a, x) + Wk.l;
      acc += wvar[3 * e] * J.x + wvar[3 * e + 1] * J.y + wvar[3 * e + 2] * J.z;
    }
    c.lamq[lane] += acc;
  }
  TS_SYNC();
  if (!wtac) return;
  for (int s = 0; s < c.nsensor; ++s) {
    const int* si = c.I + c.off_sensor + s * TSIM_SI_SIZE;
    const R* sf = c.F + c.foff_sensor + s * TSIM_SF_SIZE;
    const int t0 = ts_u(si[TSIM_SI_TAX0]), nt = ts_u(si[TSIM_SI_NTAX]), sp0 = ts_u(si[TSIM_SI_SPRIM0]), nsp = ts_u(si[TSIM_SI_NSPRIM]);
    for (int j = 0; j < nsp; ++j) {
      const int pk = ts_u(c.I[c.off_sprim + sp0 + j]);
      const int prim = ts_u(c.I[c.off_pair + pk * TSIM_PI_SIZE + TSIM_PI_PRIM]);
      const R* pf = c.F + c.foff_pair + pk * TSIM_PF_SIZE;
      TS_SYNC();
      pair_stage_value(c, pk, 0, lane == 0);
      TS_SYNC();
      const R* S = c.PP;
      PairPose<R> P;
      P.RPAd = ldm(c.PPd); P.pPAd = ldv(c.PPd + 9);
      P.RPA = ldm(S + PP_RPA); P.pPA = ldv(S + PP_PPA); P.wrel = ldv(S + PP_WREL); P.vrel = ldv(S + PP_VREL);
      R g[12];
      const bool any_live = vjp_taxels<LPE, R>(c, lane, t0, nt, prim, pf + TSIM_PF_SHAPE, sf, P, wtac, g);
      if (!any_live) continue;
      seg_sum_many<LPE, 12>(g);
      pair_stage_tangent(c, pk, 0, lane, R(1), 0);
      if (lane < nr) {
        const R* T = c.PT + lane * PT_SIZE;
        R sq_ = R(0);
#pragma unroll
        for (int e = 0; e < 12; ++e) sq_ += g[e] * T[e];
        c.lamq[lane] += sq_;
      }
      pair_stage_tangent(c, pk, 0, lane, R(1), 1);
      if (lane < nr) {
        const R* T = c.PT + lane * PT_SIZE;
        R sv_ = R(0);
#pragma unroll
        for (int e = 6; e < 12; ++e) sv_ += g[e] * T[e];
        c.lamv[lane] += sv_;
      }
    }
  }
  TS_SYNC();
}

#ifdef TS_BWD_TWO_WAVES
#define TS_KLB_BWD __launch_bounds__(TS_WAVE)
#else
#define TS_KLB_BWD TS_KLB
#endif
template <class R, int NRM, bool EXPJ, int LPE, bool POLICY = false, class MS = void>
__global__ void TS_KLB_BWD k_backward(BwdArgs<R> a) {
// ... 122 lines not shown
```

tactilesimulation_amd/csrc/tsim_launch.h:

```cpp
#pragma once
#include <type_traits>
#include "tsim_kernels.h"
#include "tsim_param_grad.h"
#include "tsim_tangent.h"
#include "tsim_tangent_closed.h"
#include "tsim_frame_jacobian.h"
#include "tsim_tactile_jacobian.h"
#include "tsim_param_jacobian.h"
#include "tsim_static_pusher.h"

enum TsKernel { TS_K_FORWARD, TS_K_BACKWARD, TS_K_BACKWARD_Z, TS_K_DEBUG_EVAL, TS_K_PARAM_GRAD, TS_K_PARAM_GRAD_BODY, TS_K_FRAME_RECORDS,
                TS_K_CLOSED_BACKWARD_Z,
                TS_K_TANGENT,
                TS_K_TANGENT_BODY,
                TS_K_CLOSED_TANGENT,
                TS_K_FRAME_JACOBIAN,
                TS_K_TACTILE_JACOBIAN,
                TS_K_PARAM_JACOBIAN };
enum { TS_KM_GENERIC = 0, TS_KM_STATIC = 1, TS_KM_PARAM = 2 };
using TsParamPusher = TsParam<TsStaticPusher>;

struct TsPlan {
  int kernel = TS_K_FORWARD, variant = TS_KM_GENERIC;
  int nrm = 8; bool expj = false; int lpe = TS_WAVE;
  bool policy = false;
  bool default_opts = false;
  bool frame_rec = false;
  unsigned grid = 0; size_t lds = 0;
  bool fused = false;
};

template <class MS> constexpr int ts_view_nrm() { return ts_static_nr<MS>() == 0 ? 0 : (ts_static_nr<MS>() <= 8 ? 8 : 16); }

constexpr bool ts_instantiated(int kernel, int ms_nrm, bool fp32, bool policy, bool default_opts, int nrm, bool expj, int lpe) {
  if ((expj && (nrm != 16 || lpe != 64)) || (nrm != 8 && nrm != 16) || (lpe != 16 && lpe != 32 && lpe != 64)) return false;
  if (kernel == TS_K_CLOSED_TANGENT) return ms_nrm == 0 && !policy && !default_opts && nrm == 8 && !expj;
  if (policy != (kernel == TS_K_CLOSED_BACKWARD_Z) && kernel != TS_K_FORWARD && kernel != TS_K_BACKWARD) return false;
  if (policy && (nrm != 8 || expj)) return false;
  if (ms_nrm == 0) return !default_opts && kernel != TS_K_FRAME_RECORDS;
  if (kernel == TS_K_PARAM_GRAD || kernel == TS_K_PARAM_GRAD_BODY || kernel == TS_K_TANGENT || kernel == TS_K_TANGENT_BODY || kernel == TS_K_FRAME_JACOBIAN || kernel == TS_K_TACTILE_JACOBIAN || kernel == TS_K_PARAM_JACOBIAN || nrm != ms_nrm || expj) return false;
  if (default_opts) return kernel == TS_K_FORWARD && fp32 && lpe == 16;
  if (policy || kernel == TS_K_DEBUG_EVAL) return fp32 && lpe == 16;
  return fp32 || lpe != 16;
}

template <class R, bool EXPJ, int LPE> __global__ void __launch_bounds__(TS_WAVE) k_param_grad(PgArgs<R> a);
template <class R, bool EXPJ, int LPE> __global__ void __launch_bounds__(TS_WAVE) k_param_grad_body(PgBodyArgs<R> a);
template <class R, int NRM, bool EXPJ, int LPE> __global__ void __launch_bounds__(TS_WAVE) k_tangent(TanArgs<R> a);
template <class R, int NRM, bool EXPJ, int LPE> __global__ void __launch_bounds__(TS_WAVE) k_tangent_src(TanArgs<R> a);
template <class R, bool EXPJ, int LPE> __global__ void __launch_bounds__(TS_WAVE) k_tangent_body_src(TanBodyArgs<R> a);
template <class R, int NRM, bool EXPJ, int LPE, bool SRC> __global__ void __launch_bounds__(TS_WAVE) k_closed_tangent(TanClosedArgs<R> a);

template <class R, int NRM, bool EXPJ, int LPE> __global__ void __launch_bounds__(TS_WAVE) k_frame_jacobian(FjArgs<R> a);
template <class R, int NRM, bool EXPJ, int LPE> __global__ void __launch_bounds__(TS_WAVE) k_tactile_jacobian(TjArgs<R> a);
template <class R, int NRM, bool EXPJ, int LPE> __global__ void __launch_bounds__(TS_WAVE) k_param_jacobian(PjArgs<R> a);

template <int N> using TsInt = std::integral_constant<int, N>;
template <bool B> using TsBool = std::integral_constant<bool, B>;

template <class MS, bool POLICY, class R> struct TsLaunch {
  template <int K, class F> static bool shape(const TsPlan& p, F&& f) {
    if (p.kernel != K || p.policy != POLICY) return false;
    auto at = [&](auto nrm, auto expj, auto lpe) {
      if constexpr (ts_instantiated(K, ts_view_nrm<MS>(), sizeof(R) == 4, POLICY, false, nrm, expj, lpe)) { f(nrm, expj, lpe); return true; }
      else return false;
    };
    auto lanes = [&](auto nrm, auto expj) { return p.lpe == 16 ? at(nrm, expj, TsInt<16>()) : p.lpe == 32 ? at(nrm, expj, TsInt<32>()) : p.lpe == 64 && at(nrm, expj, TsInt<64>()); };
    if (p.expj) return p.nrm == 16 && lanes(TsInt<16>(), TsBool<true>());
    return p.nrm == 8 ? lanes(TsInt<8>(), TsBool<false>()) : p.nrm == 16 && lanes(TsInt<16>(), TsBool<false>());
  }
  static bool run(const TsPlan& p, hipStream_t st, const FwdArgs<R>& a);
  static bool run(const TsPlan& p, hipStream_t st, const FwdArgs<R>& a, int fpc, TsSubRange sub);
  static bool run(const TsPlan& p, hipStream_t st, const BwdArgs<R>& a, R* zsave = nullptr);
  static bool run_closed_z(const TsPlan& p, hipStream_t st, const BwdArgs<R>& a, R* zsave);
  static bool run(const TsPlan& p, hipStream_t st, const DbgArgs<R>& a);
  static bool run(const TsPlan& p, hipStream_t st, const PgArgs<R>& a);
  static bool run(const TsPlan& p, hipStream_t st, const PgBodyArgs<R>& a);
  static bool run(const TsPlan& p, hipStream_t st, const TanArgs<R>& a);
  static bool run(const TsPlan& p, hipStream_t st, const TanBodyArgs<R>& a);
  static bool run(const TsPlan& p, hipStream_t st, const FjArgs<R>& a);
  static bool run(const TsPlan& p, hipStream_t st, const TjArgs<R>& a);
  static bool run(const TsPlan& p, hipStream_t st, const PjArgs<R>& a);
  static bool run_tangent_src(const TsPlan& p, hipStream_t st, const TanArgs<R>& a);
  static bool run_closed_tangent(const TsPlan& p, hipStream_t st, const TanClosedArgs<R>& a);
};

template <class MS, bool POLICY, class R> bool TsLaunch<MS, POLICY, R>::run(const TsPlan& p, hipStream_t st, const FwdArgs<R>& a) {
  return shape<TS_K_FORWARD>(p, [&](auto nrm, auto expj, auto lpe) {
    if constexpr (ts_instantiated(TS_K_FORWARD, ts_view_nrm<MS>(), sizeof(R) == 4, POLICY, true, nrm, expj, lpe)) {
      if (p.default_opts && p.frame_rec) {
        if constexpr (!POLICY && ts_static_fused<MS, R>()) { hipLaunchKernelGGL((k_forward_fr<R, nrm, lpe, MS>), dim3(p.grid), dim3(TS_WAVE), p.lds, st, a); return; }
      }
      if (p.default_opts) { hipLaunchKernelGGL((k_forward<R, nrm, expj, lpe, POLICY, TsDefaultOpts<MS>>), dim3(p.grid), dim3(TS_WAVE), p.lds, st, a); return; }
    }
    hipLaunchKernelGGL((k_forward<R, nrm, expj, lpe, POLICY, MS>), dim3(p.grid), dim3(TS_WAVE), p.lds, st, a);
  });
}
template <class MS, bool POLICY, class R> bool TsLaunch<MS, POLICY, R>::run(const TsPlan& p, hipStream_t st, const FwdArgs<R>& a, int fpc, TsSubRange sub) {
  if constexpr (!POLICY && ts_static_fused<MS, R>())
    return shape<TS_K_FRAME_RECORDS>(p, [&](auto, auto, auto lpe) { hipLaunchKernelGGL((k_frame_records<R, lpe, MS>), dim3(p.grid), dim3(TS_WAVE), p.lds, st, a, fpc, sub); });
  else return false;
}
template <class MS, bool POLICY, class R> bool TsLaunch<MS, POLICY, R>::run(const TsPlan& p, hipStream_t st, const BwdArgs<R>& a, R* zsave) {
  if (p.kernel == TS_K_CLOSED_BACKWARD_Z) return run_closed_z(p, st, a, zsave);
  if (p.kernel == TS_K_BACKWARD_Z)
    return shape<TS_K_BACKWARD_Z>(p, [&](auto nrm, auto expj, auto lpe) { hipLaunchKernelGGL((k_backward_z<R, nrm, expj, lpe, POLICY, MS>), dim3(p.grid), dim3(TS_WAVE), p.lds, st, a, zsave); });
  return shape<TS_K_BACKWARD>(p, [&](auto nrm, auto expj, auto lpe) { hipLaunchKernelGGL((k_backward<R, nrm, expj, lpe, POLICY, MS>), dim3(p.grid), dim3(TS_WAVE), p.lds, st, a); });
}
template <class MS, bool POLICY, class R> bool TsLaunch<MS, POLICY, R>::run_closed_z(const TsPlan& p, hipStream_t st, const BwdArgs<R>& a, R* zsave) {
  return shape<TS_K_CLOSED_BACKWARD_Z>(p, [&](auto nrm, auto expj, auto lpe) { hipLaunchKernelGGL((k_closed_backward_z<R, nrm, expj, lpe, MS>), dim3(p.grid), dim3(TS_WAVE), p.lds, st, a, zsave); });
}
template <class MS, bool POLICY, class R> bool TsLaunch<MS, POLICY, R>::run(const TsPlan& p, hipStream_t st, const DbgArgs<R>& a) {
  return shape<TS_K_DEBUG_EVAL>(p, [&](auto, auto, auto lpe) { hipLaunchKernelGGL((k_debug_eval<R, lpe, MS>), dim3(p.grid), dim3(TS_WAVE), p.lds, st, a); });
}
template <class MS, bool POLICY, class R> bool TsLaunch<MS, POLICY, R>::run(const TsPlan& p, hipStream_t st, const PgArgs<R>& a) {
  return shape<TS_K_PARAM_GRAD>(p, [&](auto, auto expj, auto lpe) { hipLaunchKernelGGL((k_param_grad<R, expj, lpe>), dim3(p.grid), dim3(TS_WAVE), p.lds, st, a); });
}
template <class MS, bool POLICY, class R> bool TsLaunch<MS, POLICY, R>::run(const TsPlan& p, hipStream_t st, const PgBodyArgs<R>& a) {
  return shape<TS_K_PARAM_GRAD_BODY>(p, [&](auto, auto expj, auto lpe) { hipLaunchKernelGGL((k_param_grad_body<R, expj, lpe>), dim3(p.grid), dim3(TS_WAVE), p.lds, st, a); });
}
template <class MS, bool POLICY, class R> bool TsLaunch<MS, POLICY, R>::run(const TsPlan& p, hipStream_t st, const TanArgs<R>& a) {
  return shape<TS_K_TANGENT>(p, [&](auto nrm, auto expj, auto lpe) { hipLaunchKernelGGL((k_tangent<R, nrm, expj, lpe>), dim3(p.grid), dim3(TS_WAVE), p.lds, st, a); });
}
template <class MS, bool POLICY, class R> bool TsLaunch<MS, POLICY, R>::run(const TsPlan& p, hipStream_t st, const TanBodyArgs<R>& a) {
  return shape<TS_K_TANGENT_BODY>(p, [&](auto, auto expj, auto lpe) { hipLaunchKernelGGL((k_tangent_body_src<R, expj, lpe>), dim3(p.grid), dim3(TS_WAVE), p.lds, st, a); });
}
template <class MS, bool POLICY, class R> bool TsLaunch<MS, POLICY, R>::run(const TsPlan& p, hipStream_t st, const FjArgs<R>& a) {
  return shape<TS_K_FRAME_JACOBIAN>(p, [&](auto nrm, auto expj, auto lpe) { hipLaunchKernelGGL((k_frame_jacobian<R, nrm, expj, lpe>), dim3(p.grid), dim3(TS_WAVE), p.lds, st, a); });
}
template <class MS, bool POLICY, class R> bool TsLaunch<MS, POLICY, R>::run(const TsPlan& p, hipStream_t st, const TjArgs<R>& a) {
  return shape<TS_K_TACTILE_JACOBIAN>(p, [&](auto nrm, auto expj, auto lpe) { hipLaunchKernelGGL((k_tactile_jacobian<R, nrm, expj, lpe>), dim3(p.grid), dim3(TS_WAVE), p.lds, st, a); });
}
template <class MS, bool POLICY, class R> bool TsLaunch<MS, POLICY, R>::run(const TsPlan& p, hipStream_t st, const PjArgs<R>& a) {
  return shape<TS_K_PARAM_JACOBIAN>(p, [&](auto nrm, auto expj, auto lpe) { hipLaunchKernelGGL((k_param_jacobian<R, nrm, expj, lpe>), dim3(p.grid), dim3(TS_WAVE), p.lds, st, a); });
}
template <class MS, bool POLICY, class R> bool TsLaunch<MS, POLICY, R>::run_tangent_src(const TsPlan& p, hipStream_t st, const TanArgs<R>& a) {
  return shape<TS_K_TANGENT>(p, [&](auto nrm, auto expj, auto lpe) { hipLaunchKernelGGL((k_tangent_src<R, nrm, expj, lpe>), dim3(p.grid), dim3(TS_WAVE), p.lds, st, a); });
}
template <class MS, bool POLICY, class R> bool TsLaunch<MS, POLICY, R>::run_closed_tangent(const TsPlan& p, hipStream_t st, const TanClosedArgs<R>& a) {
  return shape<TS_K_CLOSED_TANGENT>(p, [&](auto nrm, auto expj, auto lpe) {
    if (a.src) hipLaunchKernelGGL((k_closed_tangent<R, nrm, expj, lpe, true>), dim3(p.grid), dim3(TS_WAVE), p.lds, st, a);
    else hipLaunchKernelGGL((k_closed_tangent<R, nrm, expj, lpe, false>), dim3(p.grid), dim3(TS_WAVE), p.lds, st, a);
  });
}

template <bool POLICY, class R, class A, class... Z> bool ts_launch(const TsPlan& p, hipStream_t st, const A& a, Z... z) {
  if (p.variant == TS_KM_STATIC) return TsLaunch<TsStaticPusher, POLICY, R>::run(p, st, a, z...);
  if (p.variant == TS_KM_PARAM) return TsLaunch<TsParamPusher, POLICY, R>::run(p, st, a, z...);
  return TsLaunch<void, POLICY, R>::run(p, st, a, z...);
}
extern template struct TsLaunch<TsStaticPusher, false, float>;
extern template struct TsLaunch<TsStaticPusher, false, double>;
extern template struct TsLaunch<TsStaticPusher, true, float>;
extern template struct TsLaunch<TsStaticPusher, true, double>;
extern template struct TsLaunch<TsParamPusher, false, float>;
extern template struct TsLaunch<TsParamPusher, false, double>;
extern template struct TsLaunch<TsParamPusher, true, float>;
extern template struct TsLaunch<TsParamPusher, true, double>;
extern template bool TsLaunch<void, false, float>::run(const TsPlan&, hipStream_t, const PgArgs<float>&);
extern template bool TsLaunch<void, false, double>::run(const TsPlan&, hipStream_t, const PgArgs<double>&);
extern template bool TsLaunch<void, false, float>::run(const TsPlan&, hipStream_t, const PgBodyArgs<float>&);
extern template bool TsLaunch<void, false, double>::run(const TsPlan&, hipStream_t, const PgBodyArgs<double>&);
extern template bool TsLaunch<void, false, float>::run(const TsPlan&, hipStream_t, const TanArgs<float>&);
extern template bool TsLaunch<void, false, double>::run(const TsPlan&, hipStream_t, const TanArgs<double>&);
extern template bool TsLaunch<void, false, float>::run(const TsPlan&, hipStream_t, const TanBodyArgs<float>&);
extern template bool TsLaunch<void, false, double>::run(const TsPlan&, hipStream_t, const TanBodyArgs<double>&);
extern template bool TsLaunch<void, false, float>::run(const TsPlan&, hipStream_t, const FjArgs<float>&);
extern template bool TsLaunch<void, false, double>::run(const TsPlan&, hipStream_t, const FjArgs<double>&);
extern template bool TsLaunch<void, false, float>::run(const TsPlan&, hipStream_t, const TjArgs<float>&);
extern template bool TsLaunch<void, false, double>::run(const TsPlan&, hipStream_t, const TjArgs<double>&);
extern template bool TsLaunch<void, false, float>::run(const TsPlan&, hipStream_t, const PjArgs<float>&);
extern template bool TsLaunch<void, false, double>::run(const TsPlan&, hipStream_t, const PjArgs<double>&);
extern template bool TsLaunch<void, false, float>::run_tangent_src(const TsPlan&, hipStream_t, const TanArgs<float>&);
extern template bool TsLaunch<void, false, double>::run_tangent_src(const TsPlan&, hipStream_t, const TanArgs<double>&);
extern template bool TsLaunch<void, false, float>::run_closed_tangent(const TsPlan&, hipStream_t, const TanClosedArgs<float>&);
extern template bool TsLaunch<void, false, double>::run_closed_tangent(const TsPlan&, hipStream_t, const TanClosedArgs<double>&);
extern template bool TsLaunch<void, true, float>::run_closed_z(const TsPlan&, hipStream_t, const BwdArgs<float>&, float*);
extern template bool TsLaunch<void, true, double>::run_closed_z(const TsPlan&, hipStream_t, const BwdArgs<double>&, double*);
void ts_closed_slots_launch(int32_t* slots, int nframes, hipStream_t st);
```

tactilesimulation_amd/host/batch.py:

```python
import ctypes as C

import numpy as np
import torch

from . import capi
from ..model.compiler import CompiledModel, load_model


def _ptr(t):
    return C.c_void_p(t.data_ptr()) if t is not None else None


class BatchSim:
    def __init__(self, model, batch_size, device="cuda:0", dtype=torch.float32, tape_capacity=512):
        if isinstance(model, str):
            model = load_model(model)
        assert isinstance(model, CompiledModel)
        self.model = model
        self.device = torch.device(device)
        if self.device.type != "cuda":
            raise RuntimeError("BatchSim needs a GPU device (got %s); the HIP path has no CPU fallback" % device)
        if dtype not in (torch.float32, torch.float64):
            raise ValueError("dtype must be float32 or float64")
        self.dtype = dtype
# ... 183 lines not shown
            ins.append(t if t.numel() else None)
        ndir = 1 if ndir is None else ndir
        if not 1 <= ndir <= self.TANGENT_MAX_DIR:
            raise ValueError("tangent_episode: 1 .. %d directions per launch, got %d" % (self.TANGENT_MAX_DIR, ndir))
        new = lambda n, d: torch.empty((ndir, n, self.B, d), device=self.device, dtype=self.dtype)
        o = {"dq": new(T, self.ndof_r)}
        if want_qd:
            o["dqd"] = new(T, self.ndof_r)
        if want_var and self.ndof_var:
            o["dvar"] = new(T, self.ndof_var)
        if want_tactile and self.ndof_tactile:
            o["dtactile"] = new(nm, self.ndof_tactile)
        capi.check(capi.lib().tsim_tangent_episode(self._h, T, int(num_steps), ndir, _ptr(slots), _ptr(ins[0]), _ptr(ins[1]), _ptr(ins[2]), _ptr(ins[3]),
                                                   _ptr(o["dq"]), _ptr(o.get("dqd")), _ptr(o.get("dvar")), _ptr(o.get("dtactile")), self._stream()))
        return o

    def frame_jacobians(self, num_frames, num_steps, want_A=True, want_B=True, want_var=False):
        T = int(num_frames)
        n2 = 2 * self.ndof_r
        new = lambda r, c: torch.empty((T, self.B, r, c), device=self.device, dtype=self.dtype)
        o = {}
        if want_A:
            o["A"] = new(n2, n2)
        if want_B:
            o["B"] = new(n2, self.ndof_u)
        if want_var and self.ndof_var:
            o["Jvar"] = new(self.ndof_var, self.ndof_r)
        capi.check(capi.lib().tsim_frame_jacobians(self._h, T, int(num_steps), _ptr(o.get("A")), _ptr(o.get("B")), _ptr(o.get("Jvar")), self._stream()))
        return o

    def tactile_jacobians(self, num_frames, num_steps, tactile_mask=None):
        T = int(num_frames)
        slots, nm = self._tactile_slots(T, tactile_mask)
        if nm < 1:
            raise ValueError("tactile_jacobians: the mask has no masked frame")
        Ct = torch.empty((nm, self.B, 2 * self.ndof_r, self.ndof_tactile), device=self.device, dtype=self.dtype)
        capi.check(capi.lib().tsim_tactile_jacobians(self._h, T, int(num_steps), _ptr(slots), _ptr(Ct), self._stream()))
        return Ct

    PARAM_JACOBIAN_MAX_COLS = 32

    def param_jacobians(self, num_frames, num_steps, cols, want_E=True, want_tactile=False, tactile_mask=None):
        T = int(num_frames)
        o = {}
        ncols, carr = 0, None
        if want_E:
            cols = [int(x) for x in cols]
            ncols = len(cols)
            carr = (C.c_int32 * max(ncols, 1))(*cols)
            o["E"] = torch.empty((T, self.B, 2 * self.ndof_r, ncols), device=self.device, dtype=self.dtype)
        slots = None
        if want_tactile:
            slots, nm = self._tactile_slots(T, tactile_mask)
            if nm < 1:
                raise ValueError("param_jacobians: the mask has no masked frame")
            o["Ft"] = torch.empty((nm, self.B, 4, self.ndof_tactile), device=self.device, dtype=self.dtype)
        capi.check(capi.lib().tsim_param_jacobians(self._h, T, int(num_steps), ncols, carr, _ptr(slots), _ptr(o.get("E")), _ptr(o.get("Ft")), self._stream()))
        return o

    def get_state(self):
        q, qd =self.empty(self.ndof_r), self.empty(self.ndof_r)
        capi.check(capi.lib().tsim_get_state(self._h, _ptr(q), _ptr(qd), self._stream()))
        return q, qd

    def readout(self, want_var=True, want_tactile=True):
        var = self.empty(self.ndof_var) if (want_var and self.ndof_var) else None
        tac = self.empty(self.ndof_tactile) if (want_tactile and self.ndof_tactile) else None
        if var is not None or tac is not None:
            capi.check(capi.lib().tsim_readout(self._h, _ptr(var), _ptr(tac), self._stream()))
        return var, tac

    def backward_steps(self, n, df_dq=None, df_dvar=None, df_dtactile=None, all_steps=False):
        mul = n if all_steps else 1
        a = self._chk(df_dq, mul * self.ndof_r, "df_dq")
        b = self._chk(df_dvar, mul * self.ndof_var, "df_dvar") if self.ndof_var else None
        c = self._chk(df_dtactile, mul * self.ndof_tactile, "df_dtactile") if self.ndof_tactile else None
        du = self.empty(n, self.ndof_u)
        capi.check(capi.lib().tsim_backward_steps(self._h, int(n), int(bool(all_steps)), _ptr(a), _ptr(b), _ptr(c), _ptr(du),
                                                  self._stream()))
        return du

    def get_adjoint(self):
        a, b = self.empty(self.ndof_r), self.empty(self.ndof_r)
        capi.check(capi.lib().tsim_get_adjoint(self._h, _ptr(a), _ptr(b), self._stream()))
        return a, b

    def tape_len(self):
        return capi.lib().tsim_tape_len(self._h)

    def cache_save(self):
        capi.check(capi.lib().tsim_cache_save(self._h, self._stream()))

    def cache_pop(self):
        capi.check(capi.lib().tsim_cache_pop(self._h, self._stream()))

    def cache_clear(self):
        capi.check(capi.lib().tsim_cache_clear(self._h))

    def cache_reserve(self, depth):
        capi.check(capi.lib().tsim_cache_reserve(self._h, int(depth)))

    def cache_depth(self):
        return capi.lib().tsim_cache_depth(self._h)

    def debug_eval(self, q1, q0, qd0, u, cycles=False):
        q1, q0, qd0 = (self._chk(x, self.ndof_r, "q") for x in (q1, q0, qd0))
        u = self._chk(u, self.ndof_u, "u")
        g, H = self.empty(self.ndof_r), self.empty(self.ndof_r, self.ndof_r)
        cyc = torch.zeros(self.B, 32, device=self.device, dtype=torch.int64) if cycles else None
        capi.check(capi.lib().tsim_debug_eval(self._h, _ptr(q1), _ptr(q0), _ptr(qd0), _ptr(u), _ptr(g), _ptr(H), _ptr(cyc),
                                              self._stream()))
        return (g, H, cyc) if cycles else (g, H)

    def branch_signature(self, t_first=0, n=None):
        n = self.tape_len() - t_first if n is None else int(n)
        out = torch.empty((n, self.B, 2), device=self.device, dtype=torch.int32)
        capi.check(capi.lib().tsim_debug_signature(self._h, int(t_first), n, _ptr(out), self._stream()))
        return out.to(torch.int64) & 0xFFFFFFFF

    def last_evals(self):
        out = np.zeros(self.B, dtype=np.int32)
        capi.check(capi.lib().tsim_last_evals(self._h, out.ctypes.data_as(capi._ip)))
        return out

    def last_helper_trials(self):
        out = np.zeros(self.B, dtype=np.int32)
        capi.check(capi.lib().tsim_last_helper_trials(self._h, out.ctypes.data_as(capi._ip)))
        return out

    def last_gnorm(self):
        out = np.zeros(self.B, dtype=np.float32)
        capi.check(capi.lib().tsim_last_gnorm(self._h, out.ctypes.data_as(C.POINTER(C.c_float))))
        return out

    def set_solver_options(self, cross_kinks=None, eval_budget=0):
        if cross_kinks is None:
            cross_kinks = self.dtype == torch.float32
        capi.check(capi.lib().tsim_set_solver_options(self._h, int(bool(cross_kinks)), int(eval_budget)))

    def set_lanes_per_env(self, lanes):
        capi.check(capi.lib().tsim_set_lanes_per_env(self._h, int(lanes)))

    def static_model(self):
        return capi.lib().tsim_static_model(self._h)

    def set_static(self, allow):
        capi.check(capi.lib().tsim_set_static(self._h, int(bool(allow))))

    def kernel_variant(self):
        return capi.lib().tsim_kernel_variant(self._h).decode()

    OPT_PAIR_CULL, OPT_VALUE_TRIALS, OPT_TRIAL_HELPERS, OPT_VALUE_FIRST, OPT_CROSS_KINKS, OPT_EVAL_BUDGET, OPT_ALL_DEFAULT, OPT_FRAME_RECORDS = 1, 2, 3, 4, 5, 6, 7, 8
    OPT_FORWARD_SPLIT = 9

    def set_option(self, option, value):
        capi.check(capi.lib().tsim_set_option(self._h, int(option), int(value)))

    def get_option(self, option):
        return capi.lib().tsim_get_option(self._h, int(option))

    KERNEL_KINDS = ("k_forward", "k_taxels", "k_backward")

    def kernel_timing(self, enable=True):
        capi.check(capi.lib().tsim_kernel_timing(self._h, int(bool(enable))))

    def kernel_times(self):
        ms, n = (C.c_double * 3)(), (C.c_int32 * 3)()
        capi.check(capi.lib().tsim_kernel_times(self._h, ms, n))
        return {k: (float(ms[i]), int(n[i])) for i, k in enumerate(self.KERNEL_KINDS)}

    def launch_info(self):
        out = (C.c_int32 * 4)()
        capi.lib().tsim_launch_info(self._h, out)
        return {"lds_bytes": out[0], "threads": out[1], "blocks": out[2], "lanes_per_env": out[3]}

    def tangent_launch_info(self, ndir=8, with_dtables=True):
        out = (C.c_int32 * 4)()
        capi.check(capi.lib().tsim_tangent_launch_info(self._h, int(ndir), int(bool(with_dtables)), out))
        return {"lds_bytes": out[0], "threads": out[1], "blocks": out[2], "lanes_per_env": out[3]}

    def frame_jacobians_launch_info(self):
        out = (C.c_int32 * 4)()
        capi.check(capi.lib().tsim_frame_jacobians_launch_info(self._h, out))
        return {"lds_bytes": out[0], "threads": out[1], "blocks": out[2], "lanes_per_env": out[3]}

    def tactile_jacobians_launch_info(self):
        out = (C.c_int32 * 4)()
        capi.check(capi.lib().tsim_tactile_jacobians_launch_info(self._h, out))
        return {"lds_bytes": out[0], "threads": out[1], "blocks": out[2], "lanes_per_env": out[3]}

    def param_jacobians_launch_info(self):
        out = (C.c_int32 * 4)()
        capi.check(capi.lib().tsim_param_jacobians_launch_info(self._h, out))
        return {"lds_bytes": out[0], "threads": out[1], "blocks": out[2], "lanes_per_env": out[3]}
```

tactilesimulation_amd/host/buildhash.py:

```python
import hashlib
import os


def digest(paths, flags=()):
    h = hashlib.sha256()
    for f in flags:
        h.update(f.encode() + b"\0")
    for p in paths:
        h.update(os.path.basename(p).encode() + b"\0")
        with open(p, "rb") as fh:
            h.update(fh.read())
    return h.hexdigest()


def sidecar(lib):
    return lib + ".buildhash"


def read(lib):
    try:
        return open(sidecar(lib)).read().strip()
    except OSError:
        return None


def write(lib, value):
    with open(sidecar(lib), "w") as fh:
        fh.write(value + "\n")


_PKG = os.path.dirname(os.path.dirname(os.path.abspath(__file__)))
CSRC = os.path.join(_PKG, "csrc")
INCLUDE = os.path.join(os.path.dirname(_PKG), "include")
HIP_SO = os.path.join(CSRC, "libtsim_hip.so")
HIP_FLAGS = ["--offload-arch=gfx950", "-Os", "-std=c++17", "-fPIC", "-fno-slp-vectorize", "-mllvm", "-amdgpu-function-calls=false",
             "-mllvm", "-amdgpu-sched-strategy=iterative-ilp"]
HIP_UNITS = [("tsim_hip.hip", []), ("tsim_static_pusher.hip", ["-ffinite-math-only", "-fno-signed-zeros", "-O2"]),
             ("tsim_param_pusher.hip", ["-ffinite-math-only", "-fno-signed-zeros", "-O2"]),
             ("tsim_static_pusher_policy.hip", ["-ffinite-math-only", "-fno-signed-zeros"]),
             ("tsim_param_pusher_policy.hip", ["-ffinite-math-only", "-fno-signed-zeros"]),
             ("tsim_param_grad.hip", []),
             ("tsim_param_grad_body.hip", []),
             ("tsim_closed_backward_z.hip", []),
             ("tsim_tangent.hip", []),
             ("tsim_tangent_body.hip", []),
             ("tsim_tangent_closed.hip", []),
             ("tsim_frame_jacobian.hip", []),
             ("tsim_tactile_jacobian.hip", []),
             ("tsim_param_jacobian.hip", []),
             ("tsim_model.cpp", ["-ffp-contract=off"])]
HOST_FLAGS = ["-O2", "-std=c++17", "-fPIC"]


def hip_build_commands(hipcc, out_so=None):
    out_so = out_so or HIP_SO
    bdir = os.path.join(CSRC, "build")
    cmds, objs = [], []
    for src, extra in HIP_UNITS:
        obj = os.path.join(bdir, os.path.splitext(src)[0] + ".o")
        cmds.append(([hipcc] + (HIP_FLAGS if src.endswith(".hip") else HOST_FLAGS) + extra + ["-c", os.path.join(CSRC, src), "-o", obj], CSRC))
        objs.append(obj)
    cmds.append(([hipcc, "--offload-arch=gfx950", "-shared", "-fPIC", "-o", out_so] + objs, CSRC))
    return bdir, cmds


def hip_sources():
    srcs = sorted(f for f in os.listdir(CSRC) if f.endswith((".hip", ".h", ".cpp")))
    return [os.path.join(CSRC, f) for f in srcs] + [os.path.join(INCLUDE, f) for f in ("tsim.h", "tsim_blob.h", "tsim_env.h", "tsim_model.h")]


def hip_digest():
    return digest(hip_sources(), HIP_FLAGS + HOST_FLAGS + [u + ":" + " ".join(f) for u, f in HIP_UNITS])


KERNELS_JSON = HIP_SO + ".kernels.json"
_LLVM = "/opt/rocm/lib/llvm/bin"


def write_kernel_table(lib=None, out=None):
    import json
    import re
    import shutil
    import subprocess
    import tempfile
    lib, out = lib or HIP_SO, out or KERNELS_JSON
    tmp = tempfile.mkdtemp(prefix="tsim_kt_")
    try:
        shutil.copy(lib, os.path.join(tmp, "lib.so"))
        subprocess.run([os.path.join(_LLVM, "llvm-objdump"), "--offloading", "lib.so"], cwd=tmp, stdout=subprocess.DEVNULL, stderr=subprocess.DEVNULL, check=True)
        table = {}
        for f in sorted(os.listdir(tmp)):
            if "amdgcn" not in f:
                continue
            notes = subprocess.run([os.path.join(_LLVM, "llvm-readelf"), "--notes", f], cwd=tmp, capture_output=True, text=True, check=True).stdout
            syms = subprocess.run([os.path.join(_LLVM, "llvm-readelf"), "-sW", f], cwd=tmp, capture_output=True, text=True, check=True).stdout
            size = {}
            for line in syms.splitlines():
                t = line.split()
                if len(t) >= 8 and t[3] == "FUNC":
                    size[t[7]] = int(t[2])
            for blk in re.split(r"\n\s*- \.agpr_count:", notes)[1:]:
                blk = ".agpr_count:" + blk
                g = lambda k: re.search(r"\.%s:\s+(\S+)" % k, blk)
                name = g("name")
                if not name:
                    continue
                name = name.group(1)
                rec = {k: int(g(k).group(1)) for k in ("agpr_count", "vgpr_count", "sgpr_count", "vgpr_spill_count", "sgpr_spill_count", "group_segment_fixed_size",
                                                        "private_segment_fixed_size", "max_flat_workgroup_size") if g(k)}
                rec["code_bytes"] = size.get(name)
                table[name] = rec
        with open(out, "w") as fh:
            json.dump(table, fh, indent=0, sort_keys=True)
        return table
    finally:
        shutil.rmtree(tmp, ignore_errors=True)


def kernel_name(kernel, dtype, nr, has_exp, lanes, variant, policy=False, default_opts=False):
    nrm, expj, lpe = (16, True, 64) if has_exp else ((8 if nr <= 8 else 16), False, lanes)
    if variant != "generic":
        nrm = 8
    ms = {"generic": ("v", "void"), "static:pusher": ("14TsStaticPusher", "TsStaticPusher"), "param:pusher": ("7TsParamI14TsStaticPusherE", "TsParam<TsStaticPusher>")}[variant]
    if default_opts and kernel == "k_forward" and variant != "generic" and dtype == "f32" and lpe == 16:
        ms = ("13TsDefaultOptsI%sE" % ms[0], "TsDefaultOpts<%s>" % ms[1])
    r = {"f32": ("f", "float"), "f64": ("d", "double")}[dtype]
    if kernel == "k_frame_records":
        return ("_Z15k_frame_recordsI%sLi%dE%sEv7FwdArgsIT_Ei10TsSubRange" % (r[0], lpe, ms[0]), "k_frame_records<%s, LPE=%d, %s>" % (r[1], lpe, ms[1]))
    if kernel == "k_forward_fr":
        return ("_Z12k_forward_frI%sLi%dELi%dE%sEv7FwdArgsIT_E" % (r[0], nrm, lpe, ms[0]), "k_forward_fr<%s, NRM=%d, LPE=%d, %s>" % (r[1], nrm, lpe, ms[1]))
    if kernel == "k_closed_backward_z":
        back = {"generic": 1, "static:pusher": 2, "param:pusher": 4}[variant]
        return ("_Z19k_closed_backward_zI%sLi%dELb%dELi%dE%sEv7BwdArgsIT_EPS%d_" % (r[0], nrm, int(expj), lpe, ms[0], back),
                "k_closed_backward_z<%s, NRM=%d, EXPJ=%s, LPE=%d, %s>" % (r[1], nrm, str(expj).lower(), lpe, ms[1]))
    args = {"k_forward": "7FwdArgs", "k_backward": "7BwdArgs"}[kernel]
    mangled = "_Z%d%sI%sLi%dELb%dELi%dELb%dE%sEv%sIT_E" % (len(kernel), kernel, r[0], nrm, int(expj), lpe, int(policy), ms[0], args)
    return mangled, "%s<%s, NRM=%d, EXPJ=%s, LPE=%d, POLICY=%s, %s>" % (kernel, r[1], nrm, str(expj).lower(), lpe, str(policy).lower(), ms[1])
```

Baseline: 34.68 million.

## Add one-thread-per-record output kernel and size taxel LDS dynamically

Adds k_record_outputs, which reconstructs each frame record's link poses, variables and sensor pose records with one thread per (frame, env) instead of the lane-group k_frame_records. It becomes the default readout path when frame records are enabled, with an env var to restore the old path. The small taxel kernel also moves from fixed-size static shared arrays to dynamically sized LDS and merges its staging loops, dropping two barriers. The per-thread kernel may raise register pressure but avoids cross-lane synchronisation and improves occupancy for the readout stage.

New measurement: 34.87 million, median of 6. About the same (+0.6%).

```diff
diff --git a/include/tsim.h b/include/tsim.h
--- a/include/tsim.h
+++ b/include/tsim.h
@@ -95,7 +95,7 @@
 int tsim_set_static(tsim_batch* b, int allow);
 const char* tsim_kernel_variant(const tsim_batch* b);
 enum { TSIM_OPT_PAIR_CULL = 1, TSIM_OPT_VALUE_TRIALS = 2, TSIM_OPT_TRIAL_HELPERS = 3, TSIM_OPT_VALUE_FIRST = 4, TSIM_OPT_CROSS_KINKS = 5, TSIM_OPT_EVAL_BUDGET = 6,
-       TSIM_OPT_ALL_DEFAULT = 7, TSIM_OPT_FRAME_RECORDS = 8, TSIM_OPT_FORWARD_SPLIT = 9 };
+       TSIM_OPT_ALL_DEFAULT = 7, TSIM_OPT_FRAME_RECORDS = 8, TSIM_OPT_FORWARD_SPLIT = 9, TSIM_OPT_RECORD_OUTPUTS = 10 };
 int tsim_set_option(tsim_batch* b, int option, int value);
 int tsim_get_option(const tsim_batch* b, int option);
 
diff --git a/tactilesimulation_amd/csrc/tsim_batch.h b/tactilesimulation_amd/csrc/tsim_batch.h
--- a/tactilesimulation_amd/csrc/tsim_batch.h
+++ b/tactilesimulation_amd/csrc/tsim_batch.h
@@ -69,11 +69,12 @@
   hipStream_t split_st = nullptr;
   hipEvent_t split_fork = nullptr;
   hipEvent_t split_join = nullptr;
+  int last_record_outputs = 0;
   int last_fwd_split = 0;
   int value_trials = 2;
   int trial_helpers = 1;
   int value_first = 1;
-  bool ab_no_episode_lpt = false, ab_inkernel_readout = false, ab_no_free_run = false, ab_lockstep = false, ab_taxels_per_record = false, ab_no_envtab_cpt = false, ab_no_default_opts = false, ab_inkernel_frame_out = false; int ab_bwd_lpe = 0, ab_lpt_deal = 2;
+  bool ab_no_episode_lpt = false, ab_inkernel_readout = false, ab_no_free_run = false, ab_lockstep = false, ab_taxels_per_record = false, ab_no_envtab_cpt = false, ab_no_default_opts = false, ab_inkernel_frame_out = false, ab_frame_records_slots = false; int ab_bwd_lpe = 0, ab_lpt_deal = 2;
   int pair_cull = 1;
   int static_id = 0, static_exact = 0, env_struct_ok = 0, no_static = 0;
   DevBuf dKmask, dFlag;
diff --git a/tactilesimulation_amd/csrc/tsim_hip.hip b/tactilesimulation_amd/csrc/tsim_hip.hip
--- a/tactilesimulation_amd/csrc/tsim_hip.hip
+++ b/tactilesimulation_amd/csrc/tsim_hip.hip
@@ -196,47 +196,63 @@
 }
 
 enum { TXS_RPB = 16, TXS_MAXK = 8, TXS_MAXS = 4, TXS_MAX_TAXELS = 1024 };
+template <class R> struct TxsLds {
+  int oD, oC, oSf, oShape, oP, oX, oI, bytes;
+  __host__ __device__ TxsLds(int ntax, int nspt, int nsensor) {
+    int o = 0;
+    oD = o; o += TXS_RPB * nspt * TP_D_SIZE * (int)sizeof(double);
+    oC = o; o += TXS_RPB * nspt * 4 * (int)sizeof(R);
+    oSf = o; o += TXS_RPB * nsensor * TSIM_SF_SIZE * (int)sizeof(R);
+    oShape = o; o += TXS_RPB * nspt * 4 * (int)sizeof(R);
+    oP = o; o += TXS_RPB * nspt * TP_R_SIZE * (int)sizeof(R);
+    oX = o; o += 3 * ntax * (int)sizeof(R);
+    oI = o; o += (3 * nsensor + nspt + 2 * TXS_RPB) * (int)sizeof(int);
+    bytes = o;
+  }
+};
 template <class R>
 __global__ void __launch_bounds__(256) k_taxels_small(TaxArgs<R> a, int nrec, TsSubRange sub) {
   const int rec0 = blockIdx.x * TXS_RPB, nr_ = min((int)TXS_RPB, nrec - rec0);
   const int ntax = a.ntax, nsensor = a.nsensor, nspt = a.nspt;
-  __shared__ int sEnd[TXS_MAXS], sKb[TXS_MAXS], sNsp[TXS_MAXS], sPrim[TXS_MAXK], sPair[TXS_MAXK], sSlot[TXS_RPB], sEnv[TXS_RPB], sRec[TXS_RPB];
-  __shared__ R sSf[TXS_RPB][TXS_MAXS * TSIM_SF_SIZE], sShape[TXS_RPB][TXS_MAXK * 4], sP[TXS_RPB][TXS_MAXK * TP_R_SIZE];
-  __shared__ double sD[TXS_RPB][TXS_MAXK * TP_D_SIZE];
-  __shared__ __attribute__((aligned(16))) R sC[TXS_RPB][TXS_MAXK * 4];
-  __shared__ R sX[3 * TXS_MAX_TAXELS];
+  extern __shared__ __attribute__((aligned(16))) unsigned char txs_raw[];
+  const TxsLds<R> L(ntax, nspt, nsensor);
+  double* sD = reinterpret_cast<double*>(txs_raw + L.oD);
+  R* sC = reinterpret_cast<R*>(txs_raw + L.oC);
+  R* sSf = reinterpret_cast<R*>(txs_raw + L.oSf);
+  R* sShape = reinterpret_cast<R*>(txs_raw + L.oShape);
+  R* sP = reinterpret_cast<R*>(txs_raw + L.oP);
+  R* sX = reinterpret_cast<R*>(txs_raw + L.oX);
+  int* sEnd = reinterpret_cast<int*>(txs_raw + L.oI); int* sKb = sEnd + nsensor; int* sNsp = sKb + nsensor; int* sPrim = sNsp + nsensor;
+  int* sSlot = sPrim + nspt; int* sEnv = sSlot + TXS_RPB;
+  const int nP = nspt * TP_R_SIZE, nD = nspt * TP_D_SIZE, nSf = nsensor * TSIM_SF_SIZE, nSh = nspt * 4;
+  auto rec_of = [&](int r, int& fr) { fr = (rec0 + r) / sub.n; const int ei = sub.e0 + (rec0 + r) - fr * sub.n; return sub.order ? sub.order[ei] : ei; };
   const R* tax = a.F + a.foff_taxel;
+  const int* TT = a.I + a.tt_off;
+  for (int i = threadIdx.x; i < nr_; i += 256) { int fr; const int env = rec_of(i, fr); sSlot[i] = a.tac_slot ? a.tac_slot[fr] : fr; sEnv[i] = env; }
+  for (int i = threadIdx.x; i < nr_ * nP; i += 256) { const int r = i / nP, e = i - r * nP; int fr; const int env = rec_of(r, fr); sP[i] = a.poseR[(size_t)(fr * a.B + env) * nP + e]; }
+  for (int i = threadIdx.x; i < nr_ * nD; i += 256) { const int r = i / nD, e = i - r * nD; int fr; const int env = rec_of(r, fr); sD[i] = a.poseD[(size_t)(fr * a.B + env) * nD + e]; }
+  for (int i = threadIdx.x; i < nr_ * nSf; i += 256) {
+    const int r = i / nSf, e = i - r * nSf; int fr;
+    const R* F = a.Fenv ? a.Fenv + (size_t)rec_of(r, fr) * a.fstride : a.F;
+    sSf[i] = F[a.foff_sensor + e];
+  }
+  for (int i = threadIdx.x; i < nr_ * nSh; i += 256) {
+    const int r = i / nSh, e = i - r * nSh; int fr;
+    const R* F = a.Fenv ? a.Fenv + (size_t)rec_of(r, fr) * a.fstride : a.F;
+    sShape[i] = F[a.foff_pair + TT[3 * nsensor + 2 * (e >> 2) + 1] * TSIM_PF_SIZE + TSIM_PF_SHAPE + (e & 3)];
+  }
   for (int i = threadIdx.x; i < 3 * ntax; i += 256) sX[i] = tax[i];
-  const int* TT = a.I + a.tt_off;
   for (int i = threadIdx.x; i < nsensor; i += 256) { sEnd[i] = TT[3 * i]; sKb[i] = TT[3 * i + 1]; sNsp[i] = TT[3 * i + 2]; }
-  for (int i = threadIdx.x; i < nspt; i += 256) { sPrim[i] = TT[3 * nsensor + 2 * i]; sPair[i] = TT[3 * nsensor + 2 * i + 1]; }
-  for (int i = threadIdx.x; i < nr_; i += 256) {
-    const int fr = (rec0 + i) / sub.n, ei = sub.e0 + (rec0 + i) - fr * sub.n, env = sub.order ? sub.order[ei] : ei;
-    sSlot[i] = a.tac_slot ? a.tac_slot[fr] : fr; sEnv[i] = env; sRec[i] = fr * a.B + env;
-  }
+  for (int i = threadIdx.x; i < nspt; i += 256) sPrim[i] = TT[3 * nsensor + 2 * i];
   __syncthreads();
-  for (int i = threadIdx.x; i < nr_ * nspt * TP_R_SIZE; i += 256) { const int r = i / (nspt * TP_R_SIZE), e = i % (nspt * TP_R_SIZE); sP[r][e] = a.poseR[(size_t)sRec[r] * nspt * TP_R_SIZE + e]; }
-  for (int i = threadIdx.x; i < nr_ * nspt * TP_D_SIZE; i += 256) { const int r = i / (nspt * TP_D_SIZE), e = i % (nspt * TP_D_SIZE); sD[r][e] = a.poseD[(size_t)sRec[r] * nspt * TP_D_SIZE + e]; }
-  for (int i = threadIdx.x; i < nr_ * nsensor * TSIM_SF_SIZE; i += 256) {
-    const int r = i / (nsensor * TSIM_SF_SIZE), e = i % (nsensor * TSIM_SF_SIZE);
-    const R* F = a.Fenv ? a.Fenv + (size_t)sEnv[r] * a.fstride : a.F;
-    sSf[r][e] = F[a.foff_sensor + e];
-  }
-  __syncthreads();
-  for (int i = threadIdx.x; i < nr_ * nspt * 4; i += 256) {
-    const int r = i / (nspt * 4), e = i % (nspt * 4);
-    const R* F = a.Fenv ? a.Fenv + (size_t)sEnv[r] * a.fstride : a.F;
-    sShape[r][e] = F[a.foff_pair + sPair[e >> 2] * TSIM_PF_SIZE + TSIM_PF_SHAPE + (e & 3)];
-  }
-  __syncthreads();
-  for (int i = threadIdx.x; i < nr_ * nspt; i += 256) { const int r = i / nspt, k = i % nspt; taxel_bound<R>(sP[r] + k * TP_R_SIZE, sPrim[k], sShape[r] + k * 4, sC[r] + 4 * k); }
+  for (int i = threadIdx.x; i < nr_ * nspt; i += 256) { const int r = i / nspt, k = i - r * nspt; taxel_bound<R>(sP + r * nP + k * TP_R_SIZE, sPrim[k], sShape + r * nSh + k * 4, sC + r * nSh + 4 * k); }
   __syncthreads();
   for (int item = threadIdx.x; item < nr_ * ntax; item += 256) {
     const int r = item / ntax, t = item - r * ntax;
     const int tslot = sSlot[r];
     if (tslot < 0) continue;
     R* out = a.tac_out + ((size_t)tslot * a.B + sEnv[r]) * 3 * ntax;
-    taxel_eval<R>(t, mk3<R>(sX[t], sX[t + ntax], sX[t + 2 * ntax]), nsensor, sEnd, sKb, sNsp, sPrim, sSf[r], sShape[r], sP[r], sD[r], sC[r], tax, ntax, out);
+    taxel_eval<R>(t, mk3<R>(sX[t], sX[t + ntax], sX[t + 2 * ntax]), nsensor, sEnd, sKb, sNsp, sPrim, sSf + r * nSf, sShape + r * nSh, sP + r * nP, sD + r * nD, sC + r * nSh, tax, ntax, out);
   }
 }
 
@@ -618,7 +634,9 @@
   if (taxels_small(b, nrec)) {
     TaxArgs<R> t{b->dI, (const R*)b->dF, (const R*)b->dFenv, b->nfrec, (const R*)poseR, poseD, b->nspt, (R*)tac_out, 0, b->B, tac_slot,
                  b->ntax, b->I[TSIM_IH_NSENSOR], b->I[TSIM_IH_FOFF_SENSOR], b->I[TSIM_IH_FOFF_PAIR], b->I[TSIM_IH_FOFF_TAXEL], b->tt_off};
-    hipLaunchKernelGGL(k_taxels_small<R>, dim3((unsigned)((nrec + TXS_RPB - 1) / TXS_RPB)), dim3(256), 0, st, t, (int)nrec, sub ? *sub : all);
+    const TxsLds<R> lds(t.ntax, t.nspt, t.nsensor);
+    if (lds.bytes > 64 * 1024) (void)hipFuncSetAttribute(reinterpret_cast<const void*>(&k_taxels_small<R>), hipFuncAttributeMaxDynamicSharedMemorySize, lds.bytes);
+    hipLaunchKernelGGL(k_taxels_small<R>, dim3((unsigned)((nrec + TXS_RPB - 1) / TXS_RPB)), dim3(256), (size_t)lds.bytes, st, t, (int)nrec, sub ? *sub : all);
     HIPCHK(hipGetLastError());
     return 0;
   }
@@ -668,8 +686,15 @@
   plan.frame_rec = frame_rec;
   b->last_frame_rec = !frame_rec ? 0 : (plan.frame_rec && plan.default_opts) ? 2 : 1;
   const int ns_ = TS_WAVE / plan.lpe;
+  const bool by_lane = frame_rec && !b->ab_frame_records_slots;
+  b->last_record_outputs = !frame_rec ? 0 : by_lane ? 2 : 1;
   auto frame_records = [&](hipStream_t s, const TsSubRange& sub) {
     TsPlan p = fr_plan;
+    if (by_lane) {
+      p.kernel = TS_K_RECORD_OUTPUTS; p.lds = 0;
+      p.grid = (unsigned)(((long long)nframes * sub.n + TS_WAVE - 1) / TS_WAVE);
+      return ts_launch<false, R>(p, s, a, sub);
+    }
     const int nblk = (sub.n + ns_ - 1) / ns_, chunks = std::max(1, std::min(nframes, b->n_simd / std::max(nblk, 1))), fpc = (nframes + chunks - 1) / chunks;
     p.grid = (unsigned)(nblk * ((nframes + fpc - 1) / fpc));
     return ts_launch<false, R>(p, s, a, fpc, sub);
@@ -687,7 +712,7 @@
       return 0;
     };
     auto read_out = [&](hipStream_t s, const TsSubRange& sub) -> int {
-      if (!frame_records(s, sub)) return fail("no k_frame_records instantiation for the launch plan");
+      if (!frame_records(s, sub)) return fail("no k_frame_records / k_record_outputs instantiation for the launch plan");
       HIPCHK(hipGetLastError());
       return launch_taxels<R>(b, b->fposeR, b->fposeD, nframes, tac_slot, tac_out, s, &sub);
     };
@@ -719,7 +744,7 @@
     if (defer) {
       KtScope kt_(b, TSIM_KT_TAXELS, st);
       if (frame_rec) {
-        if (!frame_records(st, TsSubRange{nullptr, 0, b->B})) return fail("no k_frame_records instantiation for the launch plan");
+        if (!frame_records(st, TsSubRange{nullptr, 0, b->B})) return fail("no k_frame_records / k_record_outputs instantiation for the launch plan");
         HIPCHK(hipGetLastError());
       }
       if (launch_taxels<R>(b, b->fposeR, b->fposeD, nframes, tac_slot, tac_out, st)) return 1;
@@ -974,6 +999,7 @@
   b->ab_taxels_per_record = getenv("TSIM_TAXELS_PER_RECORD") != nullptr; b->ab_no_envtab_cpt = getenv("TSIM_NO_ENVTAB_CPT") != nullptr;
   b->value_first = getenv("TSIM_NO_VALUE_FIRST") ? 0 : 1;
   b->ab_inkernel_frame_out = getenv("TSIM_INKERNEL_FRAME_OUT") != nullptr;
+  b->ab_frame_records_slots = getenv("TSIM_FRAME_RECORDS_SLOTS") != nullptr;
   if (const char* e = getenv("TSIM_VALUE_TRIALS")) b->value_trials = std::max(0, atoi(e));
   if (const char* e = getenv("TSIM_LPE")) { const int v = atoi(e); if (v == 16 || v == 32 || v == 64) b->lpe_forced = v; }
   b->cross_kinks = dtype == TSIM_F32 ? 1 : 0;
@@ -1100,6 +1126,7 @@
   if (option == TSIM_OPT_ALL_DEFAULT) return default_options(b) ? 1 : 0;
   if (option == TSIM_OPT_FRAME_RECORDS) return b->last_frame_rec;
   if (option == TSIM_OPT_FORWARD_SPLIT) return b->last_fwd_split;
+  if (option == TSIM_OPT_RECORD_OUTPUTS) return b->last_record_outputs;
   return -1;
 }
 int tsim_set_solver_options(tsim_batch* b, int cross_kinks, int eval_budget) {
diff --git a/tactilesimulation_amd/csrc/tsim_kernels.h b/tactilesimulation_amd/csrc/tsim_kernels.h
--- a/tactilesimulation_amd/csrc/tsim_kernels.h
+++ b/tactilesimulation_amd/csrc/tsim_kernels.h
@@ -495,6 +495,104 @@
   }
 }
 
+__device__ __forceinline__ float ts_opaque(float x) { asm volatile("" : "+v"(x)); return x; }
+__device__ __forceinline__ double ts_opaque(double x) { asm volatile("" : "+v"(x)); return x; }
+template <class T> __device__ __forceinline__ V3<T> ts_opaque(V3<T> v) { return mk3<T>(ts_opaque(v.x), ts_opaque(v.y), ts_opaque(v.z)); }
+template <class T> __device__ __forceinline__ M3<T> ts_opaque(M3<T> A) {
+#pragma unroll
+  for (int e = 0; e < 9; ++e) A.m[e] = ts_opaque(A.m[e]);
+  return A;
+}
+template <class R> struct TsLinkRec { M3<double> Rd; V3<double> pd; M3<R> XR; V3<R> Xp; S6<R> V; };
+template <class R, class MS, int LINK>
+__device__ __forceinline__ void ts_ro_link_recs(const TsLinkState<R>* st, const TsLinkTmp<R>* tmp, TsLinkRec<R>* lr) {
+  if constexpr (LINK == 0) {
+    const double one = ts_opaque(1.0), zero = ts_opaque(0.0);
+    const R oneR = ts_opaque(R(1)), zeroR = ts_opaque(R(0));
+    lr[0].Rd = M3<double>{{one, zero, zero, zero, one, zero, zero, zero, one}}; lr[0].pd = mk3<double>(zero, zero, zero);
+    lr[0].XR = M3<R>{{oneR, zeroR, zeroR, zeroR, oneR, zeroR, zeroR, zeroR, oneR}}; lr[0].Xp = mk3<R>(zeroR, zeroR, zeroR);
+    lr[0].V = mk6<R>(mk3<R>(zeroR, zeroR, zeroR), mk3<R>(zeroR, zeroR, zeroR));
+    ts_ro_link_recs<R, MS, 1>(st, tmp, lr);
+  } else if constexpr (LINK <= TsTopo<MS>::NL) {
+    lr[LINK].Rd = ts_opaque(st[LINK].Rd); lr[LINK].pd = ts_opaque(st[LINK].pd);
+    lr[LINK].XR = ts_opaque(tmp[LINK].XR); lr[LINK].Xp = ts_opaque(tmp[LINK].Xp);
+    lr[LINK].V = mk6<R>(ts_opaque(st[LINK].V.a), ts_opaque(st[LINK].V.l));
+    ts_ro_link_recs<R, MS, LINK + 1>(st, tmp, lr);
+  }
+}
+template <class R, class MS, int E>
+__device__ __forceinline__ void ts_ro_variables(const R* F, const TsLinkRec<R>* lr, R* o) {
+  if constexpr (E < MS::Iv(TSIM_IH_NVAR)) {
+    constexpr int l = MS::Iv(MS::Iv(TSIM_IH_OFF_VAR) + E * TSIM_VI_SIZE + TSIM_VI_LINK);
+    const V3<R> x = mulMv(lr[l].XR, ldv(F + MS::Iv(TSIM_IH_FOFF_VAR) + E * TSIM_VF_SIZE)) + lr[l].Xp;
+    o[3 * E] = x.x; o[3 * E + 1] = x.y; o[3 * E + 2] = x.z;
+    ts_ro_variables<R, MS, E + 1>(F, lr, o);
+  }
+}
+template <class R, class MS, int S, int J, int K>
+__device__ __forceinline__ void ts_ro_pose_records(const R* F, const TsLinkRec<R>* lr, R* poseR, double* poseD) {
+  if constexpr (S < MS::Iv(TSIM_IH_NSENSOR)) {
+    constexpr int so = MS::Iv(TSIM_IH_OFF_SENSOR) + S * TSIM_SI_SIZE, nsp = MS::Iv(so + TSIM_SI_NSPRIM), sp0 = MS::Iv(so + TSIM_SI_SPRIM0);
+    if constexpr (J < nsp) {
+      constexpr int pk = MS::Iv(MS::Iv(TSIM_IH_OFF_SPRIM) + sp0 + J), po = MS::Iv(TSIM_IH_OFF_PAIR) + pk * TSIM_PI_SIZE;
+      constexpr int la = MS::Iv(po + TSIM_PI_LINKA), lb = MS::Iv(po + TSIM_PI_LINKB);
+      const R* pf = F + MS::Iv(TSIM_IH_FOFF_PAIR) + pk * TSIM_PF_SIZE;
+      const M3<double> RBd = lr[lb].Rd;
+      const M3<double> RPd = mulMM(RBd, ldm_as<double>(pf + TSIM_PF_R));
+      const V3<double> pPd = mulMv(RBd, ldv_as<double>(pf + TSIM_PF_P)) + lr[lb].pd;
+      const M3<double> RPAd = mulMtM(RPd, lr[la].Rd);
+      const V3<double> pPAd = mulMtv(RPd, lr[la].pd - pPd);
+      const M3<R> RP = cvtm<R>(RPd);
+      const V3<R> pP = cvt3<R>(pPd);
+      const S6<R> Vrel = to_frame(RP, pP, lr[la].V - lr[lb].V);
+      double* D = poseD + K * TP_D_SIZE;
+      R* P = poseR + K * TP_R_SIZE;
+      stm(D, RPAd); stv(D + 9, pPAd);
+      stm(P + PP_RPA, cvtm<R>(RPAd)); stv(P + PP_PPA, cvt3<R>(pPAd)); st6(P + PP_WREL, Vrel);
+      ts_ro_pose_records<R, MS, S, J + 1, K + 1>(F, lr, poseR, poseD);
+    } else ts_ro_pose_records<R, MS, S + 1, 0, K>(F, lr, poseR, poseD);
+  }
+}
+template <class R, class MS>
+__global__ void __launch_bounds__(TS_WAVE) k_record_outputs(FwdArgs<R> a, TsSubRange sub) {
+  using T = TsTopo<MS>;
+  static_assert(PP_RPA == 0 && PP_PPA == 9 && PP_WREL == 12 && PP_VREL == 15 && TP_R_SIZE == 18, "the pose record is the head of the staged pair record");
+  constexpr int nr = T::NR;
+  const long long nrec = (long long)a.nframes * sub.n, g_ = (long long)blockIdx.x * TS_WAVE + threadIdx.x;
+  const bool live = g_ < nrec;
+  const long long g = live ? g_ : nrec - 1;
+  const int f = (int)(g / sub.n), ei = sub.e0 + (int)(g - (long long)f * sub.n);
+  const int env = sub.order ? sub.order[ei] : ei;
+  const int tslot = a.tac_slot ? a.tac_slot[f] : f;
+  const int REC = ts_rec(nr, MS::Iv(TSIM_IH_NU), (int)sizeof(R), a.tk);
+  const R* st_ = a.tape + ((size_t)(a.t0 + (f + 1) * a.nsub) * a.B + env) * REC;
+  double qD[nr]; R qd[nr], qa[nr];
+#pragma unroll
+  for (int k = 0; k < nr; ++k) { qD[k] = rec_q(st_)[k]; qd[k] = st_[rec_qd<R>(nr) + k]; qa[k] = R(0); }
+  const R* F = a.Fenv ? a.Fenv + (size_t)env * a.fstride : a.F;
+  Ctx<R> c{};
+  c.F = F; c.qD = qD; c.qd = qd; c.qa = qa;
+  TsLinkState<R> st[T::NL + 1];
+  TsLinkTmp<R> tmp[T::NL + 1];
+  S6<R> Wk = zero6<R>(), dFl[T::NL + 1];
+  ts_l_level<R, MS, false, false, 0, 0>(c, 0, R(0), R(0), R(0), st, tmp, Wk, dFl);
+  TsLinkRec<R> lr[T::NL + 1];
+  ts_ro_link_recs<R, MS, 0>(st, tmp, lr);
+  if (!live) return;
+  const size_t o = ((size_t)f * a.B + env) * nr;
+#pragma unroll
+  for (int k = 0; k < nr; ++k) {
+    if (a.q_out) a.q_out[o + k] = (R)qD[k];
+    if (a.qd_out) a.qd_out[o + k] = qd[k];
+  }
+  constexpr int nvar = MS::Iv(TSIM_IH_NVAR);
+  if (a.var_out) ts_ro_variables<R, MS, 0>(F, lr, a.var_out + ((size_t)f * a.B + env) * 3 * nvar);
+  if (a.fposeR && tslot >= 0) {
+    const size_t rec = ((size_t)f * a.B + env) * a.nspt;
+    ts_ro_pose_records<R, MS, 0, 0, 0>(F, lr, a.fposeR + rec * TP_R_SIZE, a.fposeD + rec * TP_D_SIZE);
+  }
+}
+
 
 template <class R, int LPE, class MS> __device__ __forceinline__ void ts_static_output_vjp(const Ctx<R>& c, int lane, const R* wvar, const R* wtac);
 template <class R> struct BwdArgs {
diff --git a/tactilesimulation_amd/csrc/tsim_launch.h b/tactilesimulation_amd/csrc/tsim_launch.h
--- a/tactilesimulation_amd/csrc/tsim_launch.h
+++ b/tactilesimulation_amd/csrc/tsim_launch.h
@@ -16,7 +16,8 @@
                 TS_K_CLOSED_TANGENT,
                 TS_K_FRAME_JACOBIAN,
                 TS_K_TACTILE_JACOBIAN,
-                TS_K_PARAM_JACOBIAN };
+                TS_K_PARAM_JACOBIAN,
+                TS_K_RECORD_OUTPUTS };
 enum { TS_KM_GENERIC = 0, TS_KM_STATIC = 1, TS_KM_PARAM = 2 };
 using TsParamPusher = TsParam<TsStaticPusher>;
 
@@ -34,6 +35,7 @@
 
 constexpr bool ts_instantiated(int kernel, int ms_nrm, bool fp32, bool policy, bool default_opts, int nrm, bool expj, int lpe) {
   if ((expj && (nrm != 16 || lpe != 64)) || (nrm != 8 && nrm != 16) || (lpe != 16 && lpe != 32 && lpe != 64)) return false;
+  if (kernel == TS_K_RECORD_OUTPUTS) return ms_nrm != 0 && !policy && !default_opts && nrm == ms_nrm && !expj && lpe == 64;
   if (kernel == TS_K_CLOSED_TANGENT) return ms_nrm == 0 && !policy && !default_opts && nrm == 8 && !expj;
   if (policy != (kernel == TS_K_CLOSED_BACKWARD_Z) && kernel != TS_K_FORWARD && kernel != TS_K_BACKWARD) return false;
   if (policy && (nrm != 8 || expj)) return false;
@@ -71,6 +73,7 @@
   }
   static bool run(const TsPlan& p, hipStream_t st, const FwdArgs<R>& a);
   static bool run(const TsPlan& p, hipStream_t st, const FwdArgs<R>& a, int fpc, TsSubRange sub);
+  static bool run(const TsPlan& p, hipStream_t st, const FwdArgs<R>& a, TsSubRange sub);
   static bool run(const TsPlan& p, hipStream_t st, const BwdArgs<R>& a, R* zsave = nullptr);
   static bool run_closed_z(const TsPlan& p, hipStream_t st, const BwdArgs<R>& a, R* zsave);
   static bool run(const TsPlan& p, hipStream_t st, const DbgArgs<R>& a);
@@ -100,6 +103,13 @@
   if constexpr (!POLICY && ts_static_fused<MS, R>())
     return shape<TS_K_FRAME_RECORDS>(p, [&](auto, auto, auto lpe) { hipLaunchKernelGGL((k_frame_records<R, lpe, MS>), dim3(p.grid), dim3(TS_WAVE), p.lds, st, a, fpc, sub); });
   else return false;
+}
+template <class MS, bool POLICY, class R> bool TsLaunch<MS, POLICY, R>::run(const TsPlan& p, hipStream_t st, const FwdArgs<R>& a, TsSubRange sub) {
+  if constexpr (!POLICY && ts_static_fused<MS, R>() && ts_instantiated(TS_K_RECORD_OUTPUTS, ts_view_nrm<MS>(), sizeof(R) == 4, POLICY, false, ts_view_nrm<MS>(), false, 64)) {
+    if (p.kernel != TS_K_RECORD_OUTPUTS || p.policy) return false;
+    hipLaunchKernelGGL((k_record_outputs<R, MS>), dim3(p.grid), dim3(TS_WAVE), 0, st, a, sub);
+    return true;
+  } else return false;
 }
 template <class MS, bool POLICY, class R> bool TsLaunch<MS, POLICY, R>::run(const TsPlan& p, hipStream_t st, const BwdArgs<R>& a, R* zsave) {
   if (p.kernel == TS_K_CLOSED_BACKWARD_Z) return run_closed_z(p, st, a, zsave);
diff --git a/tactilesimulation_amd/host/batch.py b/tactilesimulation_amd/host/batch.py
--- a/tactilesimulation_amd/host/batch.py
+++ b/tactilesimulation_amd/host/batch.py
@@ -359,6 +359,7 @@
 
     OPT_PAIR_CULL, OPT_VALUE_TRIALS, OPT_TRIAL_HELPERS, OPT_VALUE_FIRST, OPT_CROSS_KINKS, OPT_EVAL_BUDGET, OPT_ALL_DEFAULT, OPT_FRAME_RECORDS = 1, 2, 3, 4, 5, 6, 7, 8
     OPT_FORWARD_SPLIT = 9
+    OPT_RECORD_OUTPUTS = 10
 
     def set_option(self, option, value):
         capi.check(capi.lib().tsim_set_option(self._h, int(option), int(value)))
diff --git a/tactilesimulation_amd/host/buildhash.py b/tactilesimulation_amd/host/buildhash.py
--- a/tactilesimulation_amd/host/buildhash.py
+++ b/tactilesimulation_amd/host/buildhash.py
@@ -127,6 +127,8 @@
     r = {"f32": ("f", "float"), "f64": ("d", "double")}[dtype]
     if kernel == "k_frame_records":
         return ("_Z15k_frame_recordsI%sLi%dE%sEv7FwdArgsIT_Ei10TsSubRange" % (r[0], lpe, ms[0]), "k_frame_records<%s, LPE=%d, %s>" % (r[1], lpe, ms[1]))
+    if kernel == "k_record_outputs":
+        return ("_Z16k_record_outputsI%s%sEv7FwdArgsIT_E10TsSubRange" % (r[0], ms[0]), "k_record_outputs<%s, %s>" % (r[1], ms[1]))
     if kernel == "k_forward_fr":
         return ("_Z12k_forward_frI%sLi%dELi%dE%sEv7FwdArgsIT_E" % (r[0], nrm, lpe, ms[0]), "k_forward_fr<%s, NRM=%d, LPE=%d, %s>" % (r[1], nrm, lpe, ms[1]))
     if kernel == "k_closed_backward_z":
```
